# lbarseghyan/diffusion-models

Measured on AMD Instinct MI355X. Metric: sampled images/sec, 32x32 U-Net (dim 64, mults 1-2-4-8), DDPM-1000, higher is better.
Workload: dtype f32; 1 GPU; ddpm1000_32x32_unet64_b256_per_gpu; sampler=p_sample_loop (DDPM), sampler_steps=1000, batch_per_gpu=256, global_batch=256, hip_graph=True, graph_captures=1, parallelism=batch-shard x1, one all-gather per sample()

## Files before the change

### diffusion-models_amd/_lib.py

```python
from __future__ import annotations

import ctypes as C
import os
from typing import Optional

_HERE = os.path.dirname(os.path.abspath(__file__))
LIB_PATH = os.environ.get("DM_LIB") or os.path.join(_HERE, "libdm_hip.so")
DM_MAX_STAGES = 8
DM_COEFS = 8
DM_EDM_COEFS = 16
EDM_HEUN, EDM_DPMPP = 0, 1
DM_CT_COEFS = 16
CT_PRED_NOISE, CT_PRED_V = 0, 1
ABI_VERSION = 9

EXPORTS = (
    "dm_last_error", "dm_abi_version",
    "dm_unet_create", "dm_unet_destroy", "dm_unet_set_param", "dm_unet_missing_params", "dm_unet_get_param_host", "dm_unet_finalize",
    "dm_unet_update_param", "dm_unet_refresh", "dm_unet_graph_captures", "dm_unet_workspace_bytes",
    "dm_unet_forward", "dm_unet_forward_masked", "dm_sample", "dm_sample_cond", "dm_sample_ex", "dm_randn",
    "dm_decoder_create", "dm_decoder_destroy", "dm_decoder_set_param", "dm_decoder_missing_params",
    "dm_decoder_finalize", "dm_decoder_forward",
    "dm_encoder_create", "dm_encoder_destroy", "dm_encoder_set_param", "dm_encoder_missing_params",
    "dm_encoder_finalize", "dm_encoder_forward",
    "dm_op_conv2d", "dm_op_downsample", "dm_op_rmsnorm", "dm_op_block", "dm_op_linear_attention",
    "dm_op_attention", "dm_op_sampler_update", "dm_op_cfg_combine",
    "dm_op_group_norm", "dm_op_vae_attention", "dm_op_vq_nearest",
    "dm_conv_create", "dm_conv_destroy", "dm_conv_forward", "dm_op_pool2d", "dm_op_resize_bilinear",
    "dm_op_copy_channels_nhwc", "dm_op_global_avgpool", "dm_op_linear",
    "dm_unet_train_enable", "dm_unet_grad_floats", "dm_unet_grads_flat", "dm_unet_train_buckets", "dm_unet_train_bucket", "dm_unet_get_grad", "dm_unet_loss_backward", "dm_unet_loss_backward_ex", "dm_unet_loss_backward_masked", "dm_op_q_sample", "dm_op_linear_bwd",
    "dm_op_offset_noise", "dm_op_cdist", "dm_op_gather_rows", "dm_op_lincomb", "dm_op_mask_mix",
    "dm_op_mse_loss", "dm_op_adam_step", "dm_op_ema_lerp",
    "dm_unet_optimizer_step", "dm_unet_train_scalar", "dm_unet_ema_update", "dm_unet_get_param", "dm_unet_set_train_tensor", "dm_unet_adam_step",
    "dm_unet_train_sync", "dm_unet_check_device_pack",
    "dm_unet_train_dropout", "dm_op_dropout_mask",
    "dm_op_conv2d_bwd", "dm_op_downsample_bwd", "dm_op_block_bwd", "dm_op_rmsnorm_bwd", "dm_op_linear_attention_bwd",
    "dm_op_attention_bwd", "dm_op_cross_attention", "dm_op_cross_attention_bwd",
    "dm_profile_enable", "dm_profile_read",
    "dm_unet_forward_ft", "dm_sample_edm",
    "dm_op_edm_churn_in", "dm_op_edm_euler", "dm_op_edm_heun", "dm_op_edm_dpmpp", "dm_op_edm_finalize",
    "dm_unet_train_enable_ft", "dm_unet_loss_backward_edm",
    "dm_op_edm_noise_in", "dm_op_edm_loss", "dm_op_sinusoid_ft_bwd",
    "dm_sample_ct", "dm_unet_loss_backward_ct", "dm_op_ct_step", "dm_op_ct_noise_in", "dm_op_ct_loss",
)


class UnetCfg(C.Structure):
    _fields_ = [
        ("dim", C.c_int32), ("init_dim", C.c_int32), ("out_dim", C.c_int32), ("channels", C.c_int32),
        ("input_channels", C.c_int32), ("n_stages", C.c_int32),
        ("dim_mults", C.c_int32 * DM_MAX_STAGES), ("full_attn", C.c_int32 * DM_MAX_STAGES),
        ("attn_heads", C.c_int32), ("attn_dim_head", C.c_int32),
        ("text_mode", C.c_int32), ("text_emb_dim", C.c_int32), ("sinusoidal_theta", C.c_float),
        ("learned_sinusoidal_dim", C.c_int32), ("attn_heads_stage", C.c_int32 * DM_MAX_STAGES),
    ]


class DecoderCfg(C.Structure):
    _fields_ = [
        ("ch", C.c_int32), ("out_ch", C.c_int32), ("n_levels", C.c_int32), ("ch_mult", C.c_int32 * DM_MAX_STAGES),
        ("num_res_blocks", C.c_int32), ("n_attn_res", C.c_int32), ("attn_resolutions", C.c_int32 * DM_MAX_STAGES),
        ("resolution", C.c_int32), ("z_channels", C.c_int32), ("embed_dim", C.c_int32),
    ]


class EncoderCfg(C.Structure):
    _fields_ = [
        ("ch", C.c_int32), ("in_channels", C.c_int32), ("n_levels", C.c_int32), ("ch_mult", C.c_int32 * DM_MAX_STAGES),
        ("num_res_blocks", C.c_int32), ("n_attn_res", C.c_int32), ("attn_resolutions", C.c_int32 * DM_MAX_STAGES),
        ("resolution", C.c_int32), ("z_channels", C.c_int32), ("embed_dim", C.c_int32), ("n_embed", C.c_int32),
        ("double_z", C.c_int32),
    ]


class SampleArgs(C.Structure):
    _fields_ = [
        ("kind", C.c_int32), ("objective", C.c_int32), ("self_condition", C.c_int32), ("n_steps", C.c_int32),
        ("times_host", C.POINTER(C.c_int64)), ("coefs_host", C.POINTER(C.c_float)),
        ("x_T", C.c_void_p), ("noise", C.c_void_p), ("seed", C.c_uint64), ("sample_offset", C.c_uint64),
        ("ctx", C.c_void_p), ("ctx_tokens", C.c_int32), ("cond_channels", C.c_int32), ("cond", C.c_void_p),
        ("out", C.c_void_p), ("all_steps", C.c_void_p),
        ("B", C.c_int32), ("H", C.c_int32), ("W", C.c_int32), ("unnormalize", C.c_int32), ("use_graph", C.c_int32),
        ("reserved_", C.c_int32), ("stream", C.c_void_p),
        ("cfg", C.c_int32), ("cfg_scale", C.c_float), ("cfg_rescaled_phi", C.c_float),
        ("cfg_keep_parallel_frac", C.c_float), ("cfg_remove_parallel", C.c_int32), ("cfg_reserved_", C.c_int32),
    ]


class EdmArgs(C.Structure):
    _fields_ = [
        ("kind", C.c_int32), ("n_steps", C.c_int32), ("table_host", C.POINTER(C.c_float)),
        ("x_init", C.c_void_p), ("noise", C.c_void_p), ("seed", C.c_uint64), ("sample_offset", C.c_uint64),
        ("out", C.c_void_p), ("sigma_init", C.c_float), ("clamp", C.c_int32),
        ("B", C.c_int32), ("H", C.c_int32), ("W", C.c_int32), ("use_graph", C.c_int32), ("stream", C.c_void_p),
    ]


class EdmTrainArgs(C.Structure):
    _fields_ = [
        ("images", C.c_void_p), ("noise", C.c_void_p), ("coef_host", C.POINTER(C.c_float)), ("coef_stride", C.c_int32),
        ("loss_scale", C.c_float), ("accumulate", C.c_int32), ("B", C.c_int32), ("H", C.c_int32), ("W", C.c_int32),
        ("loss_out_host", C.POINTER(C.c_float)), ("denoised_out", C.c_void_p), ("stream", C.c_void_p),
    ]


class CtArgs(C.Structure):
    _fields_ = [
        ("objective", C.c_int32), ("clip", C.c_int32), ("n_steps", C.c_int32), ("table_host", C.POINTER(C.c_float)),
        ("x_init", C.c_void_p), ("noise", C.c_void_p), ("seed", C.c_uint64), ("sample_offset", C.c_uint64),
        ("out", C.c_void_p), ("B", C.c_int32), ("H", C.c_int32), ("W", C.c_int32), ("use_graph", C.c_int32),
        ("stream", C.c_void_p),
    ]


class CtTrainArgs(C.Structure):
    _fields_ = [
        ("images", C.c_void_p), ("noise", C.c_void_p), ("coef_host", C.POINTER(C.c_float)), ("coef_stride", C.c_int32),
        ("objective", C.c_int32), ("loss_scale", C.c_float), ("accumulate", C.c_int32), ("B", C.c_int32), ("H", C.c_int32),
        ("W", C.c_int32), ("normalize", C.c_int32), ("loss_out_host", C.POINTER(C.c_float)), ("stream", C.c_void_p),
    ]


OBJECTIVES = {"pred_noise": 0, "pred_x0": 1, "pred_v": 2}


class ProfileRow(C.Structure):
    _fields_ = [("kernel", C.c_char * 64), ("launches", C.c_int64), ("total_ms", C.c_double),
                ("total_flops", C.c_double), ("total_bytes", C.c_double)]


_lib: Optional[C.CDLL] = None


def _declare(lib: C.CDLL) -> None:
    vp, i32, i64, u64, fp = C.c_void_p, C.c_int, C.c_int64, C.c_uint64, C.c_void_p
    lib.dm_last_error.restype = C.c_char_p
    lib.dm_last_error.argtypes = []
    lib.dm_abi_version.restype = i32
    lib.dm_unet_create.argtypes = [C.POINTER(UnetCfg), i32, C.POINTER(vp)]
    lib.dm_unet_destroy.argtypes = [vp]
    lib.dm_unet_destroy.restype = None
    lib.dm_unet_set_param.argtypes = [vp, C.c_char_p, fp, C.POINTER(i64), i32]
    lib.dm_unet_missing_params.argtypes = [vp]
    lib.dm_unet_finalize.argtypes = [vp]
    lib.dm_unet_get_param_host.argtypes = [vp, C.c_char_p, vp, i64]
    lib.dm_unet_forward.argtypes = [vp, fp, vp, fp, i32, fp, i32, i32, i32, vp]
    lib.dm_unet_forward_masked.argtypes = [vp, fp, vp, fp, i32, vp, fp, i32, i32, i32, vp]
    lib.dm_unet_update_param.argtypes = [vp, C.c_char_p, fp, C.POINTER(i64), i32]
    lib.dm_unet_refresh.argtypes = [vp]
    lib.dm_unet_graph_captures.argtypes = [vp]
    lib.dm_unet_workspace_bytes.argtypes = [vp]
    lib.dm_unet_workspace_bytes.restype = i64
    lib.dm_sample.argtypes = [vp, i32, i32, C.POINTER(i64), C.POINTER(C.c_float), fp, fp, u64, u64, fp, i32, fp, fp,
                              i32, i32, i32, i32, i32, vp]
    lib.dm_sample_cond.argtypes = [vp, i32, i32, C.POINTER(i64), C.POINTER(C.c_float), fp, fp, u64, u64, fp, i32, fp,
                                   i32, fp, fp, i32, i32, i32, i32, i32, vp]
    lib.dm_sample_ex.argtypes = [vp, C.POINTER(SampleArgs)]
    lib.dm_randn.argtypes = [fp, i64, u64, u64, u64, vp]
    lib.dm_decoder_create.argtypes = [C.POINTER(DecoderCfg), i32, C.POINTER(vp)]
    lib.dm_decoder_destroy.argtypes = [vp]
    lib.dm_decoder_destroy.restype = None
    lib.dm_decoder_set_param.argtypes = [vp, C.c_char_p, fp, C.POINTER(i64), i32]
    lib.dm_decoder_missing_params.argtypes = [vp]
    lib.dm_decoder_finalize.argtypes = [vp]
    lib.dm_decoder_forward.argtypes = [vp, fp, fp, i32, i32, i32, vp]
    lib.dm_encoder_create.argtypes = [C.POINTER(EncoderCfg), i32, C.POINTER(vp)]
    lib.dm_encoder_destroy.argtypes = [vp]
    lib.dm_encoder_destroy.restype = None
    lib.dm_encoder_set_param.argtypes = [vp, C.c_char_p, fp, C.POINTER(i64), i32]
    lib.dm_encoder_missing_params.argtypes = [vp]
    lib.dm_encoder_finalize.argtypes = [vp]
    lib.dm_encoder_forward.argtypes = [vp, fp, fp, fp, vp, i32, i32, i32, vp]
    lib.dm_op_conv2d.argtypes = [fp, i32, fp, i32, fp, fp, fp, fp, i32, i32, i32, i32, i32, i32, i32, vp]
    lib.dm_op_downsample.argtypes = [fp, i32, fp, fp, fp, i32, i32, i32, i32, vp]
    lib.dm_op_rmsnorm.argtypes = [fp, fp, fp, i32, i32, i32, i32, vp]
    lib.dm_op_block.argtypes = [fp, i32, fp, fp, fp, fp, fp, fp, i32, i32, i32, i32, vp]
    lib.dm_op_linear_attention.argtypes = [fp, fp, fp, fp, fp, fp, fp, fp, i32, i32, i32, i32, i32, i32, vp]
    lib.dm_op_attention.argtypes = [fp, fp, fp, fp, fp, fp, fp, i32, i32, i32, i32, i32, i32, vp]
    lib.dm_op_sampler_update.argtypes = [i32, i32, fp, fp, fp, C.POINTER(C.c_float), fp, fp, i64, vp]
    lib.dm_op_cfg_combine.argtypes = [fp, fp, fp, i32, i64, C.c_float, C.c_float, i32, C.c_float, vp]
    lib.dm_op_group_norm.argtypes = [fp, fp, fp, fp, i32, i32, i32, i32, C.c_float, i32, vp]
    lib.dm_op_vae_attention.argtypes = [fp, fp, fp, fp, i32, i32, i32, i32, vp]
    lib.dm_op_vq_nearest.argtypes = [fp, fp, fp, vp, i64, i32, i32, i32, vp]
    lib.dm_conv_create.argtypes = [fp, fp, i32, i32, i32, i32, i32, i32, i32, i32, i32, C.POINTER(vp)]
    lib.dm_conv_destroy.argtypes = [vp]
    lib.dm_conv_destroy.restype = None
    lib.dm_conv_forward.argtypes = [vp, fp, i32, i32, i32, i32, fp, vp]
    lib.dm_op_pool2d.argtypes = [fp, fp, i32, i32, i32, i32, i32, i32, i32, i32, vp]
    lib.dm_op_resize_bilinear.argtypes = [fp, fp, i32, i32, i32, i32, i32, i32, fp, fp, vp]
    lib.dm_op_copy_channels_nhwc.argtypes = [fp, i32, fp, i32, i32, i64, vp]
    lib.dm_op_global_avgpool.argtypes = [fp, fp, i32, i32, i32, vp]
    lib.dm_op_linear.argtypes = [fp, fp, fp, fp, i32, i32, i32, vp]
    lib.dm_unet_train_enable.argtypes = [vp]
    lib.dm_unet_grad_floats.argtypes = [vp]
    lib.dm_unet_grad_floats.restype = i64
    lib.dm_unet_get_grad.argtypes = [vp, C.c_char_p, fp, vp]
    lib.dm_unet_grads_flat.argtypes = [vp, C.POINTER(vp), C.POINTER(i64)]
    lib.dm_unet_train_buckets.argtypes = [vp, i32]
    lib.dm_unet_train_bucket.argtypes = [vp, i32, C.POINTER(i64), C.POINTER(i64), i32, vp]
    lib.dm_unet_loss_backward.argtypes = [vp, fp, C.POINTER(i64), C.POINTER(C.c_float), fp, fp, fp, i32, fp, i32, i32, i32,
                                          C.c_float, i32, C.POINTER(C.c_float), fp, i32, i32, i32, vp]
    lib.dm_unet_loss_backward_ex.argtypes = [vp, C.POINTER(TrainArgs)]
    lib.dm_unet_loss_backward_masked.argtypes = [vp, C.POINTER(TrainArgs), C.POINTER(C.c_int32)]
    lib.dm_unet_optimizer_step.argtypes = [vp, C.c_double, C.c_double, C.c_double, C.c_double, C.c_float, C.POINTER(C.c_float), vp]
    lib.dm_unet_train_scalar.argtypes = [vp, i32, fp, vp]
    lib.dm_unet_ema_update.argtypes = [vp, C.c_double, i32, vp]
    lib.dm_unet_get_param.argtypes = [vp, C.c_char_p, i32, fp, vp]
    lib.dm_unet_set_train_tensor.argtypes = [vp, C.c_char_p, i32, fp, vp]
    lib.dm_unet_adam_step.argtypes = [vp, C.c_longlong]
    lib.dm_unet_adam_step.restype = C.c_longlong
    lib.dm_unet_train_sync.argtypes = [vp]
    lib.dm_unet_train_dropout.argtypes = [vp, C.c_float, u64]
    lib.dm_op_dropout_mask.argtypes = [fp, i64, C.c_float, u64, u64, i32, vp]
    lib.dm_unet_check_device_pack.argtypes = [vp]
    lib.dm_op_q_sample.argtypes = [fp, fp, C.POINTER(C.c_float), fp, i32, i32, vp]
    lib.dm_op_offset_noise.argtypes = [fp, fp, C.c_float, i32, i32, vp]
    lib.dm_op_lincomb.argtypes = [fp, fp, C.POINTER(C.c_float), fp, i32, i64, i32, i32, vp]
    lib.dm_op_mask_mix.argtypes = [fp, fp, fp, fp, i64, vp]
    lib.dm_op_cdist.argtypes = [fp, fp, fp, i32, i32, i64, vp]
    lib.dm_op_gather_rows.argtypes = [fp, C.POINTER(i64), fp, i32, i64, vp]
    lib.dm_op_mse_loss.argtypes = [fp, fp, fp, fp, C.POINTER(C.c_float), i32, i32, C.c_float, C.c_float, fp, C.POINTER(C.c_float),
                                   fp, fp, i32, i32, vp]
    lib.dm_op_adam_step.argtypes = [fp, fp, fp, fp, i64, C.c_double, C.c_double, C.c_double, C.c_double, i32, C.c_float,
                                    C.POINTER(C.c_float), vp]
    lib.dm_op_ema_lerp.argtypes = [fp, fp, i64, C.c_double, vp]
    lib.dm_op_linear_bwd.argtypes = [fp, fp, fp, fp, fp, fp, i32, i32, i32, i32, vp]
    lib.dm_op_conv2d_bwd.argtypes = [fp, i32, fp, i32, fp, fp, fp, fp, fp, fp, i32, i32, i32, i32, i32, i32, i32, vp]
    lib.dm_op_downsample_bwd.argtypes = [fp, i32, fp, fp, fp, fp, fp, i32, i32, i32, i32, vp]
    lib.dm_op_block_bwd.argtypes = [fp, i32] + [fp] * 12 + [i32, i32, i32, i32, vp]
    lib.dm_op_rmsnorm_bwd.argtypes = [fp, fp, fp, fp, fp, i32, i32, i32, i32, vp]
    lib.dm_op_linear_attention_bwd.argtypes = [fp] * 15 + [i32] * 6 + [vp]
    lib.dm_op_attention_bwd.argtypes = [fp] * 13 + [i32] * 6 + [vp]
    lib.dm_op_cross_attention.argtypes = [fp] * 8 + [vp, fp] + [i32] * 7 + [vp]
    lib.dm_op_cross_attention_bwd.argtypes = [fp] * 8 + [vp] + [fp] * 9 + [i32] * 7 + [vp]
    lib.dm_profile_enable.argtypes = [i32]
    lib.dm_unet_forward_ft.argtypes = [vp, fp, fp, fp, i32, fp, i32, i32, i32, vp]
    lib.dm_sample_edm.argtypes = [vp, C.POINTER(EdmArgs)]
    lib.dm_op_edm_churn_in.argtypes = [fp, fp, C.POINTER(C.c_float), i32, u64, u64, u64, fp, fp, i32, i64, vp]
    lib.dm_op_edm_euler.argtypes = [fp, fp, C.POINTER(C.c_float), i32, i32, fp, fp, fp, fp, i32, i64, vp]
    lib.dm_op_edm_heun.argtypes = [fp, fp, fp, fp, C.POINTER(C.c_float), i32, i32, fp, i32, i64, vp]
    lib.dm_op_edm_dpmpp.argtypes = [fp, fp, fp, C.POINTER(C.c_float), i32, fp, i32, i64, vp]
    lib.dm_op_edm_finalize.argtypes = [fp, fp, i64, vp]
    lib.dm_unet_train_enable_ft.argtypes = [vp, i32]
    lib.dm_unet_loss_backward_edm.argtypes = [vp, C.POINTER(EdmTrainArgs)]
    lib.dm_op_edm_noise_in.argtypes = [fp, fp, C.POINTER(C.c_float), i32, fp, fp, fp, i32, i64, vp]
    lib.dm_op_edm_loss.argtypes = [fp, fp, fp, C.POINTER(C.c_float), C.c_float, fp, fp, C.POINTER(C.c_float), i32, i64, vp]
    lib.dm_op_sinusoid_ft_bwd.argtypes = [fp, fp, fp, i32, i32, i32, i32, vp]
    lib.dm_sample_ct.argtypes = [vp, C.POINTER(CtArgs)]
    lib.dm_unet_loss_backward_ct.argtypes = [vp, C.POINTER(CtTrainArgs)]
    lib.dm_op_ct_step.argtypes = [fp, fp, fp, C.POINTER(C.c_float), i32, i32, i32, u64, u64, u64, fp, fp, i32, i64, vp]
    lib.dm_op_ct_noise_in.argtypes = [fp, fp, C.POINTER(C.c_float), i32, i32, i32, fp, fp, i32, i64, vp]
    lib.dm_op_ct_loss.argtypes = [fp, fp, C.POINTER(C.c_float), C.c_float, fp, C.POINTER(C.c_float), i32, i64, vp]
    lib.dm_profile_read.argtypes = [C.POINTER(ProfileRow), i32, C.POINTER(i32)]


class TrainArgs(C.Structure):
    _fields_ = [("x_start", C.c_void_p), ("t_host", C.POINTER(C.c_int64)), ("coef_host", C.POINTER(C.c_float)),
                ("coef_stride", C.c_int), ("noise", C.c_void_p), ("noise_q", C.c_void_p), ("cond", C.c_void_p),
                ("cond_channels", C.c_int), ("ctx", C.c_void_p), ("ctx_tokens", C.c_int), ("self_cond", C.c_int),
                ("objective", C.c_int), ("loss_scale", C.c_float), ("accumulate", C.c_int),
                ("loss_out_host", C.POINTER(C.c_float)), ("model_out", C.c_void_p), ("B", C.c_int), ("H", C.c_int),
                ("W", C.c_int), ("stream", C.c_void_p), ("loss_terms", C.c_int), ("kl_scale", C.c_float)]


def load() -> C.CDLL:
    global _lib
    if _lib is not None:
        return _lib
    if not os.path.exists(LIB_PATH):
        raise RuntimeError(
            f"{LIB_PATH} not found: the HIP extension has not been built. "
            "Run `python -c 'import __graft_entry__ as g; g.build()'` (or `make -C diffusion-models_amd/csrc`). "
            "There is no CPU fallback."
        )
    lib = C.CDLL(LIB_PATH)
    _declare(lib)
    if lib.dm_abi_version() != ABI_VERSION:
        raise RuntimeError(f"libdm_hip.so ABI {lib.dm_abi_version()} != binding ABI {ABI_VERSION}; rebuild")
    _lib = lib
    return lib


def profile_enable(on: bool) -> None:
    check(load().dm_profile_enable(1 if on else 0))


def profile_read():
    rows = (ProfileRow * 64)()
    n = C.c_int(0)
    check(load().dm_profile_read(rows, 64, C.byref(n)))
    return [dict(kernel=rows[i].kernel.decode(), launches=int(rows[i].launches), total_ms=float(rows[i].total_ms),
                 total_flops=float(rows[i].total_flops), total_bytes=float(rows[i].total_bytes))
            for i in range(n.value)]


def check(rc: int) -> None:
    if rc != 0:
        msg = load().dm_last_error().decode(errors="replace")
        raise RuntimeError(f"libdm_hip: {msg}")


def ptr(t) -> Optional[int]:
    if t is None:
        return None
    assert t.is_contiguous(), "tensor must be contiguous at the C ABI"
    return t.data_ptr()
```

### diffusion-models_amd/csrc/conv_device.h

```cpp
#pragma once

#include "dm_common.h"

namespace dm {

using f32x16 = __attribute__((ext_vector_type(16))) float;

__device__ __forceinline__ void block_to_tile(const ConvGeom& g, int bid, int nblk, int& n_tile, int& pblock) {
    n_tile = bid % g.n_tiles_n;
    pblock = bid / g.n_tiles_n;
    if (g.xcd_groups > 0) {
        const int per = (nblk / g.n_tiles_n) / g.xcd_groups;
        pblock = (pblock % g.xcd_groups) * per + pblock / g.xcd_groups;
    }
}
using f32x4 = __attribute__((ext_vector_type(4))) float;
__device__ __forceinline__ f32x4 make_f32x4(float a, float b, float c, float d) { return f32x4{a, b, c, d}; }

using f32x2 = __attribute__((ext_vector_type(2))) float;
__device__ __forceinline__ f32x2 pk_add(f32x2 a, f32x2 b) {
    f32x2 d;
    asm("v_pk_add_f32 %0, %1, %2" : "=v"(d) : "v"(a), "v"(b));
    return d;
}
__device__ __forceinline__ f32x2 pk_sub(f32x2 a, f32x2 b) {
    f32x2 d;
    asm("v_pk_add_f32 %0, %1, %2 neg_lo:[0,1] neg_hi:[0,1]" : "=v"(d) : "v"(a), "v"(b));
    return d;
}
__device__ __forceinline__ f32x2 pk_mul(f32x2 a, f32x2 b) {
    f32x2 d;
    asm("v_pk_mul_f32 %0, %1, %2" : "=v"(d) : "v"(a), "v"(b));
    return d;
}
__device__ __forceinline__ f32x2 pk_fma(f32x2 a, f32x2 b, f32x2 c) {
    f32x2 d;
    asm("v_pk_fma_f32 %0, %1, %2, %3" : "=v"(d) : "v"(a), "v"(b), "v"(c));
    return d;
}
__device__ __forceinline__ f32x4 join4(f32x2 lo, f32x2 hi) { return __builtin_shufflevector(lo, hi, 0, 1, 2, 3); }
__device__ __forceinline__ f32x4 add4(f32x4 a, f32x4 b) { return join4(pk_add(a.xy, b.xy), pk_add(a.zw, b.zw)); }
__device__ __forceinline__ f32x4 sub4(f32x4 a, f32x4 b) { return join4(pk_sub(a.xy, b.xy), pk_sub(a.zw, b.zw)); }
__device__ __forceinline__ f32x4 fma4(f32x4 a, f32x2 s, f32x4 c) {
    return join4(pk_fma(a.xy, s, c.xy), pk_fma(a.zw, s, c.zw));
}

template <int CTRL>
__device__ __forceinline__ float dpp_f(float v) {
    return __builtin_bit_cast(float, __builtin_amdgcn_update_dpp(0, __builtin_bit_cast(int, v), CTRL, 0xF, 0xF, true));
}

__device__ __forceinline__ float half_wave_sum(float v) {
    v += dpp_f<0xB1>(v);
    v += dpp_f<0x4E>(v);
    v += dpp_f<0x141>(v);
    v += dpp_f<0x140>(v);
    v += __builtin_bit_cast(float, __builtin_amdgcn_ds_swizzle(__builtin_bit_cast(int, v), 0x401F));
    return v;
}

__device__ __forceinline__ __amdgpu_buffer_rsrc_t make_rsrc(const float* base, size_t bytes) {
    return __builtin_amdgcn_make_buffer_rsrc(const_cast<float*>(base), 0, (int)min(bytes, (size_t)0xFFFFFFFFu),
                                             0x00020000);
}
__device__ __forceinline__ f32x4 bufload4(__amdgpu_buffer_rsrc_t r, unsigned voff_bytes, unsigned soff_bytes) {
    return __builtin_bit_cast(f32x4, __builtin_amdgcn_raw_buffer_load_b128(r, (int)voff_bytes, (int)soff_bytes, 0));
}

__device__ __forceinline__ float fast_rcp(float x) { return __builtin_amdgcn_rcpf(x); }
__device__ __forceinline__ float fast_rsq(float x) { return __builtin_amdgcn_rsqf(x); }

#ifdef DM_STAMPS
__device__ __forceinline__ unsigned long long dm_stamp_now() {
    unsigned long long t;
    __builtin_amdgcn_sched_barrier(0);
    asm volatile("s_memtime %0\n\ts_waitcnt lgkmcnt(0)" : "=s"(t)::"memory");
    __builtin_amdgcn_sched_barrier(0);
    return t;
}
#define DM_STAMP_DECL unsigned long long st_prev = 0, st_acc[8] = {0, 0, 0, 0, 0, 0, 0, 0};
#define DM_STAMP(k) st_prev = dm_stamp_now();
#define DM_STAMP_ADD(k)                              \
    {                                                \
        unsigned long long st_now = dm_stamp_now();  \
        st_acc[k] += st_now - st_prev;               \
        st_prev = st_now;                            \
    }
#define DM_STAMP_FLUSH                                                                              \
    if (threadIdx.x == 0 && p.stamps) {                                                             \
        unsigned long long* sp_ = p.stamps + ((size_t)blockIdx.y * gridDim.x + blockIdx.x) * 8;     \
        for (int k_ = 0; k_ < 8; ++k_) sp_[k_] = st_acc[k_];                                        \
    }
#else
#define DM_STAMP_DECL
#define DM_STAMP(k)
#define DM_STAMP_ADD(k)
#define DM_STAMP_FLUSH
#endif

struct RowsEpilogue {
    int split;
    size_t M;
    int b0;
    bool uni;
    int HoWo;
    float* red;
    int rows_per_wg;
    int row_in_wg0;
    int wn;
    bool all_valid;
};

using gfloat_ptr = const float __attribute__((address_space(1)))*;
using gfloat_mptr = float __attribute__((address_space(1)))*;
__device__ __forceinline__ f32x4 gload4(gfloat_ptr base, unsigned off_floats) {
    using gchar_ptr = const char __attribute__((address_space(1)))*;
    return *(const f32x4 __attribute__((address_space(1)))*)((gchar_ptr)base + (off_floats << 2));
}
__device__ __forceinline__ void gstore4(gfloat_mptr base, unsigned off_floats, f32x4 v) {
    using gchar_ptr = char __attribute__((address_space(1)))*;
    *(f32x4 __attribute__((address_space(1)))*)((gchar_ptr)base + (off_floats << 2)) = v;
}

template <int NR, bool RES = true>
struct RowsPrefetch {
    f32x4 b4, g4, sc, sh;
    f32x4 res[RES ? NR : 1];
    unsigned off[NR];
};

template <int NR, bool RES>
__device__ __forceinline__ void rows_prefetch(const ConvParams& p, const RowsEpilogue& e, const int (&pixv)[NR], int cg,
                                              bool cvalid, RowsPrefetch<NR, RES>& f) {
    const int cgc = cvalid ? cg : 0;
#pragma unroll
    for (int j = 0; j < NR; ++j) {
        const unsigned px = (unsigned)max(pixv[j], 0);
        f.off[j] = (e.M < (1u << 24) ? __umul24(px, (unsigned)p.Cout) : px * (unsigned)p.Cout) + cgc;
    }
    if (p.partial) return;
    const int epi = p.epi;
    if (epi & EPI_BIAS) f.b4 = *reinterpret_cast<const f32x4*>(p.bias + cgc);
    if (epi & EPI_NORM) f.g4 = *reinterpret_cast<const f32x4*>(p.g + cgc);
    if ((epi & EPI_SCALE_SHIFT) && e.uni) {
        const float* sp = p.scale + (size_t)min(e.b0, p.B - 1) * p.ss_stride;
        f.sc = *reinterpret_cast<const f32x4*>(sp + cgc);
        f.sh = *reinterpret_cast<const f32x4*>(sp + p.Cout + cgc);
    }
    if constexpr (RES) {
        if (epi & EPI_RESIDUAL) {
            const gfloat_ptr rp = (gfloat_ptr)p.residual;
#pragma unroll
            for (int j = 0; j < NR; ++j) f.res[j] = gload4(rp, f.off[j]);
        }
    }
}

template <int WN, int NR, bool RES>
__device__ __forceinline__ void rows_epilogue(const ConvParams& p, const RowsEpilogue& e, f32x4 (&v)[NR],
                                              const int (&pixv)[NR], int cg, bool cvalid,
                                              const RowsPrefetch<NR, RES>& f) {
    const int lane = threadIdx.x & 63;
    const int rsub = lane >> 4;
    if (p.partial) {
        const gfloat_mptr po = (gfloat_mptr)(p.out + (size_t)e.split * e.M * p.Cout);
#pragma unroll
        for (int j = 0; j < NR; ++j)
            if (pixv[j] >= 0 && cvalid) gstore4(po, f.off[j], v[j]);
        return;
    }
    const int epi = p.epi;
    const f32x4 zero4 = make_f32x4(0.f, 0.f, 0.f, 0.f);
    if (epi & EPI_BIAS) {
#pragma unroll
        for (int j = 0; j < NR; ++j) v[j] = add4(v[j], f.b4);
    }
    if (!e.all_valid) {
#pragma unroll
        for (int j = 0; j < NR; ++j) v[j] = cvalid ? v[j] : zero4;
    }
    if (epi & EPI_NORM) {
        const float sqrtc = sqrtf((float)p.Cout);
        const f32x4 g4 = cvalid ? f.g4 * sqrtc : zero4;
        float ssv[NR];
#pragma unroll
        for (int j = 0; j < NR; ++j) {
            const f32x2 sq = pk_fma(v[j].zw, v[j].zw, pk_mul(v[j].xy, v[j].xy));
            float ss = sq.x + sq.y;
            ss += dpp_f<0xB1>(ss);
            ss += dpp_f<0x4E>(ss);
            ss += dpp_f<0x141>(ss);
            ss += dpp_f<0x140>(ss);
            ssv[j] = ss;
        }
        if constexpr (WN > 1) {
            if ((lane & 15) == 0) {
#pragma unroll
                for (int j = 0; j < NR; ++j) e.red[e.wn * e.rows_per_wg + e.row_in_wg0 + 4 * j + rsub] = ssv[j];
            }
            __syncthreads();
#pragma unroll
            for (int j = 0; j < NR; ++j) {
                float t = 0.f;
#pragma unroll
                for (int w = 0; w < WN; ++w) t += e.red[w * e.rows_per_wg + e.row_in_wg0 + 4 * j + rsub];
                ssv[j] = t;
            }
        }
#pragma unroll
        for (int j = 0; j < NR; ++j) {
            const float rn = fast_rsq(fmaxf(ssv[j], 1e-24f));
            const f32x4 gr = g4 * rn;
            v[j] = join4(pk_mul(v[j].xy, gr.xy), pk_mul(v[j].zw, gr.zw));
        }
    }
    if (epi & EPI_SCALE_SHIFT) {
        f32x4 sc = make_f32x4(1.f, 1.f, 1.f, 1.f), sh = zero4;
        if (e.uni) {
            sc = f.sc + 1.0f;
            sh = f.sh;
        }
#pragma unroll
        for (int j = 0; j < NR; ++j) {
            if (!e.uni && cvalid && pixv[j] >= 0) {
                const float* sp = p.scale + (size_t)(pixv[j] / e.HoWo) * p.ss_stride;
                sc = *reinterpret_cast<const f32x4*>(sp + cg) + 1.0f;
                sh = *reinterpret_cast<const f32x4*>(sp + p.Cout + cg);
            }
            v[j] = join4(pk_fma(v[j].xy, sc.xy, sh.xy), pk_fma(v[j].zw, sc.zw, sh.zw));
        }
    }
    if (epi & EPI_SILU) {
        const f32x2 nl2e = {-1.4426950408889634f, -1.4426950408889634f};
#pragma unroll
        for (int j = 0; j < NR; ++j) {
            const f32x2 t0 = pk_mul(v[j].xy, nl2e), t1 = pk_mul(v[j].zw, nl2e);
            f32x4 e4 = make_f32x4(__builtin_amdgcn_exp2f(t0.x), __builtin_amdgcn_exp2f(t0.y),
                                  __builtin_amdgcn_exp2f(t1.x), __builtin_amdgcn_exp2f(t1.y));
            e4 = e4 + 1.0f;
            const f32x4 r4 = make_f32x4(fast_rcp(e4.x), fast_rcp(e4.y), fast_rcp(e4.z), fast_rcp(e4.w));
            v[j] = v[j] * r4;
        }
    }
    if (epi & EPI_RELU) {
#pragma unroll
        for (int j = 0; j < NR; ++j)
            v[j] = make_f32x4(relu_f(v[j].x), relu_f(v[j].y), relu_f(v[j].z), relu_f(v[j].w));
    }
    const gfloat_mptr op = (gfloat_mptr)p.out;
#pragma unroll
    for (int j = 0; j < NR; ++j) {
        if (pixv[j] < 0 || !cvalid) continue;
        if constexpr (RES) {
            gstore4(op, f.off[j], (epi & EPI_RESIDUAL) ? add4(v[j], f.res[j]) : v[j]);
        } else {
            f32x4 r4 = v[j];
            if (epi & EPI_RESIDUAL) r4 = add4(r4, gload4((gfloat_ptr)p.residual, f.off[j]));
            gstore4(op, f.off[j], r4);
        }
    }
}

}
```

### diffusion-models_amd/csrc/dm_api.hip

```cpp
#include "../../include/dm_hip.h"
#include "dm_common.h"
#include "edm.h"
#include "ct.h"

#include <array>
#include <cmath>
#include <cstdlib>
#include <cstring>
#include <functional>
#include <map>
#include <memory>
#include <set>
#include <stdexcept>
#include <string>
#include <unordered_map>
#include <vector>

namespace dm {

static thread_local std::string g_err;
void set_error(const std::string& msg) { g_err = msg; }

namespace prof {
struct Rec {
// ... 529 lines not shown
        return 0;
    }
    std::vector<float> ssw, ssb;
    for (auto& pr : u->resnets) {
        const HostTensor& mw = P(u, pr.first + ".mlp.1.weight");
        const HostTensor& mb = P(u, pr.first + ".mlp.1.bias");
        ssw.insert(ssw.end(), mw.data.begin(), mw.data.end());
        ssb.insert(ssb.end(), mb.data.begin(), mb.data.end());
    }
    if (u->own.upload(ssw.data(), ssw.size(), &u->ss_w) || u->own.upload(ssb.data(), ssb.size(), &u->ss_b)) return 1;
    size_t ow = 0, ob = 0;
    for (auto& pr : u->resnets) {
        const HostTensor& mw = P(u, pr.first + ".mlp.1.weight");
        const HostTensor& mb = P(u, pr.first + ".mlp.1.bias");
        u->own.record_raw(pr.first + ".mlp.1.weight", u->ss_w + ow, mw.data.size());
        u->own.record_raw(pr.first + ".mlp.1.bias", u->ss_b + ob, mb.data.size());
        ow += mw.data.size();
        ob += mb.data.size();
    }
    return 0;
}

static int build_attn_body(dm_unet* u, AttnLayer& A, const std::string& p, int dim, bool full, int heads) {
    A.full = full;
    A.dim = dim;
    A.heads = heads;
    int hidden = heads * u->dh;
    if (up1(u, p + ".norm.g", &A.norm_g) || up1(u, p + ".mem_kv", &A.mem_kv)) return 1;
    conv_src(u, p + ".to_qkv.weight", "");
    if (make_conv(u->own, A.qkv, P(u, p + ".to_qkv.weight").data.data(), nullptr, 3 * hidden, dim, 0, 1, 1, 1, 0, false))
        return 1;
    if (full) {
        conv_src(u, p + ".to_out.weight", p + ".to_out.bias");
        if (make_conv(u->own, A.out, P(u, p + ".to_out.weight").data.data(), P(u, p + ".to_out.bias").data.data(), dim,
                      hidden, 0, 1, 1, 1, 0, false)) return 1;
        A.has16 = false;
        if (attn16_eligible(dim, heads, u->dh)) {
            std::vector<float> wp, wo;
            attn16_pack(P(u, p + ".to_qkv.weight").data.data(), P(u, p + ".norm.g").data.data(),
                        P(u, p + ".to_out.weight").data.data(), dim, wp, wo);
            float *dwp, *dwo;
            if (u->own.upload(wp.data(), wp.size(), &dwp) || u->own.upload(wo.data(), wo.size(), &dwo)) return 1;
            A.a16 = Attn16{dim, dwp, dwo, A.out.bias, A.mem_kv};
            A.has16 = true;
        }
    } else {
        conv_src(u, p + ".to_out.0.weight", p + ".to_out.0.bias");
        if (make_conv(u->own, A.out, P(u, p + ".to_out.0.weight").data.data(), P(u, p + ".to_out.0.bias").data.data(),
                      dim, hidden, 0, 1, 1, 1, 0, false)) return 1;
        if (up1(u, p + ".to_out.1.g", &A.out_g)) return 1;
        if (linattn_fused_eligible(dim, heads, u->dh)) {
            std::vector<float> wq, wk, wv, wo, kb;
            const HostTensor& og = P(u, p + ".to_out.1.g");
            if (linattn_fused_pack(P(u, p + ".to_qkv.weight").data.data(), P(u, p + ".norm.g").data.data(),
                                   P(u, p + ".to_out.0.weight").data.data(), P(u, p + ".mem_kv").data.data(), dim, wq,
                                   wk, wv, wo, kb)) {
                std::vector<float> ogs(og.data);
                for (float& v : ogs) v *= std::sqrt((float)dim);
                float *dq, *dk, *dv, *dwo, *dkb, *dog;
                const HostTensor& wor = P(u, p + ".to_out.0.weight");
                if (u->own.upload(wq.data(), wq.size(), &dq) || u->own.upload(wk.data(), wk.size(), &dk) ||
                    u->own.upload(wv.data(), wv.size(), &dv) || u->own.upload(wor.data.data(), wor.data.size(), &dwo) ||
                    u->own.upload(kb.data(), kb.size(), &dkb) || u->own.upload(ogs.data(), ogs.size(), &dog))
                    return 1;
                A.fused = LinAttnFused{dim, dq, dk, dv, dwo, A.out.bias, dog, dkb, A.mem_kv};
                A.has_fused = true;
            }
        }
    }
    return 0;
}

static int build_attn(dm_unet* u, AttnLayer& A, const std::string& p, int dim, bool full, int heads) {
    return weight_group(u, p, [&]() -> int { return build_attn_body(u, A, p, dim, full, heads); });
}

static int build_cross_body(dm_unet* u, CrossLayer& C, const std::string& p, int dim) {
    int inner = 4 * u->dh;
    conv_src(u, p + ".to_q.weight", "");
    if (make_conv(u->own, C.q, P(u, p + ".to_q.weight").data.data(), nullptr, inner, dim, 0, 1, 1, 1, 0, false)) return 1;
    conv_src(u, p + ".to_out.0.weight", p + ".to_out.0.bias");
    if (make_conv(u->own, C.out, P(u, p + ".to_out.0.weight").data.data(), P(u, p + ".to_out.0.bias").data.data(), dim,
                  inner, 0, 1, 1, 1, 0, false)) return 1;
    if (up1(u, p + ".to_k.weight", &C.wk) || up1(u, p + ".to_v.weight", &C.wv) || up1(u, p + ".to_out.1.g", &C.g) ||
        up1(u, p + ".to_out.0.weight", &C.wo_raw))
        return 1;
    return 0;
}

static int build_cross(dm_unet* u, CrossLayer& C, const std::string& p, int dim) {
    return weight_group(u, p, [&]() -> int { return build_cross_body(u, C, p, dim); });
}

static int build_all(dm_unet* u) {
    const dm_unet_cfg& cfg = u->cfg;
    const int n = cfg.n_stages;
    if (cfg.learned_sinusoidal_dim > 0) {
        if (weight_group(u, "time_mlp.0", [&]() -> int { return up1(u, "time_mlp.0.weights", &u->freqs); })) return 1;
    } else if (weight_group(u, "#freqs", [&]() -> int {
            int half = cfg.dim / 2;
            double k = std::log((double)cfg.sinusoidal_theta) / (half - 1);
            float kf = (float)(-k);
            std::vector<float> f(half);
            for (int i = 0; i < half; ++i) f[i] = std::exp((float)i * kf);
            return u->own.upload(f.data(), f.size(), &u->freqs);
        }))
        return 1;
    if (weight_group(u, "time_mlp", [&]() -> int {
            return up1(u, "time_mlp.1.weight", &u->tw1) || up1(u, "time_mlp.1.bias", &u->tb1) ||
                   up1(u, "time_mlp.3.weight", &u->tw2) || up1(u, "time_mlp.3.bias", &u->tb2);
        }))
        return 1;
    if (weight_group(u, "init_conv", [&]() -> int {
            conv_src(u, "init_conv.weight", "init_conv.bias");
            return make_conv(u->own, u->init_conv, P(u, "init_conv.weight").data.data(), P(u, "init_conv.bias").data.data(),
                             u->init_dim, cfg.input_channels, 0, 7, 7, 1, 3, false);
        }))
        return 1;
    int ss_off = 0;
    u->downs.resize(n);
    u->ups.resize(n);
    for (int i = 0; i < n; ++i) {
        int din = u->dims[i], dout = u->dims[i + 1];
        std::string q = idx("downs", i);
        Stage& S = u->downs[i];
        if (build_resnet(u, S.b1, q + ".0", din, 0, din, ss_off)) return 1;
        if (build_resnet(u, S.b2, q + ".1", din, 0, din, ss_off)) return 1;
        if (build_attn(u, S.attn, q + ".2", din, cfg.full_attn[i] != 0, stage_heads(cfg, i))) return 1;
        if (weight_group(u, q + ".3", [&]() -> int {
                conv_src(u, i < n - 1 ? q + ".3.1.weight" : q + ".3.weight", i < n - 1 ? q + ".3.1.bias" : q + ".3.bias");
                if (i < n - 1) {
                    return make_conv(u->own, S.resample, P(u, q + ".3.1.weight").data.data(),
                                     P(u, q + ".3.1.bias").data.data(), dout, din, 0, 2, 2, 2, 0, false);
                }
                return make_conv(u->own, S.resample, P(u, q + ".3.weight").data.data(), P(u, q + ".3.bias").data.data(),
                                 dout, din, 0, 3, 3, 1, 1, false);
            }))
            return 1;
    }
    int mid = u->dims.back();
    if (build_resnet(u, u->mid1, "mid_block1", mid, 0, mid, ss_off)) return 1;
    if (build_attn(u, u->mid_attn, "mid_attn", mid, true, stage_heads(cfg, n - 1))) return 1;
    if (build_resnet(u, u->mid2, "mid_block2", mid, 0, mid, ss_off)) return 1;
    for (int j = 0; j < n; ++j) {
        int din = u->dims[n - 1 - j], dout = u->dims[n - j];
        std::string q = idx("ups", j);
        Stage& S = u->ups[j];
        if (build_resnet(u, S.b1, q + ".0", dout, din, dout, ss_off)) return 1;
        if (build_resnet(u, S.b2, q + ".1", dout, din, dout, ss_off)) return 1;
        if (build_attn(u, S.attn, q + ".2", dout, cfg.full_attn[n - 1 - j] != 0, stage_heads(cfg, n - 1 - j))) return 1;
        if (weight_group(u, q + ".3", [&]() -> int {
                conv_src(u, j < n - 1 ? q + ".3.1.weight" : q + ".3.weight", j < n - 1 ? q + ".3.1.bias" : q + ".3.bias");
                if (j < n - 1)
                    return make_conv(u->own, S.resample, P(u, q + ".3.1.weight").data.data(),
                                     P(u, q + ".3.1.bias").data.data(), din, dout, 0, 3, 3, 1, 1, true);
                return make_conv(u->own, S.resample, P(u, q + ".3.weight").data.data(), P(u, q + ".3.bias").data.data(),
                                 din, dout, 0, 3, 3, 1, 1, false);
            }))
            return 1;
    }
    if (build_resnet(u, u->final_res, "final_res_block", u->init_dim, u->init_dim, u->init_dim, ss_off)) return 1;
    if (weight_group(u, "final_conv", [&]() -> int {
            conv_src(u, "final_conv.weight", "final_conv.bias");
            return make_conv(u->own, u->final_conv, P(u, "final_conv.weight").data.data(),
                             P(u, "final_conv.bias").data.data(), u->out_dim, u->init_dim, 0, 1, 1, 1, 0, false);
        }))
        return 1;
    u->ss_total = ss_off;
    if (build_scale_shift(u)) return 1;
    if (cfg.text_mode == DM_TEXT_CONCAT) {
        if (weight_group(u, "text_proj", [&]() -> int {
                return up1(u, "text_proj.0.weight", &u->tp_w0) || up1(u, "text_proj.0.bias", &u->tp_b0) ||
                       up1(u, "text_proj.2.weight", &u->tp_w2) || up1(u, "text_proj.2.bias", &u->tp_b2);
            }) ||
            weight_group(u, "text_concat_proj", [&]() -> int {
                return up1(u, "text_concat_proj.weight", &u->tc_w) || up1(u, "text_concat_proj.bias", &u->tc_b);
            }))
            return 1;
    } else if (cfg.text_mode == DM_TEXT_CROSS) {
        if (build_cross(u, u->cross_mid, "cross_attn", mid) || build_cross(u, u->cross_down, "cross_attn_down", mid) ||
            build_cross(u, u->cross_up, "cross_attn_up", mid))
            return 1;
    }
    return 0;
}

struct Ctx {
    dm_unet* u;
    Arena* A;
    hipStream_t s;
    int B;
    const float* ss;
    int ss_stride;
    bool dry() const { return A->dry; }
};

struct ResParts {
    const float* part;
    int nsplit;
    int64_t stride;
    const float* bias;
};

struct PlannedConv {
    ConvParams p;
    int out_h, out_w;
    int kind;
    bool in_kernel;
};

static int plan_conv(const Ctx& c, const ConvLayer& L, bool has_in1, int Hin, int Win, int epi, bool in_nchw, bool out_nchw,
                     PlannedConv& P) {
    ConvParams& p = P.p;
    p = ConvParams{};
    p.C0 = L.C0; p.C1 = L.C1;
    const int CK = conv_ck_for(L.C0, L.C1);
    p.chunks0 = (L.C0 + CK - 1) / CK;
    p.n_chunks = p.chunks0 + (L.C1 ? (L.C1 + CK - 1) / CK : 0);
    p.in_nchw = in_nchw ? 1 : 0;
    p.w = L.w; p.bias = L.bias;
    p.Cout = L.Cout; p.stride = L.stride; p.pad = L.pad;
    const int padw = L.pad_w >= 0 ? L.pad_w : L.pad;
    p.pad_w = padw;
    p.B = c.B;
    p.out_nchw = out_nchw ? 1 : 0;
    p.ss_stride = c.ss_stride;
    const bool want_norm = (epi & EPI_NORM) != 0;
    P.kind = 0;
    const bool upwino = L.up && L.wwu && !in_nchw && !out_nchw && !has_in1 && Hin % 2 == 0 && Win % 2 == 0 &&
                        upwino_shape_ok(c.B, Hin / 2, Win / 2, L.Cout, L.C0, L.C1);
    if (upwino) {
        p.fold = 0; p.fold_w_stride = 0; p.up = 1;
        p.KH = 3; p.KW = 3;
        p.Hin = Hin / 2; p.Win = Win / 2;
        p.Ho = Hin; p.Wo = Win;
        P.out_h = Hin; P.out_w = Win;
        p.w = L.wwu;
        p.chunks0 = p.n_chunks = L.C0 / 8;
        p.geo = upwino_plan(c.B, p.Hin, p.Win, L.Cout, L.C0, L.C1, true);
        P.kind = 3;
    } else if (L.fold) {
        DM_REQUIRE(!out_nchw && !in_nchw, "folded upsample conv is NHWC");
        p.fold = 1; p.fold_w_stride = L.fold_w_stride; p.up = 0;
        p.KH = 2; p.KW = 2; p.pad_w = 1;
        p.Hin = Hin / 2; p.Win = Win / 2;
        p.Ho = p.Hin; p.Wo = p.Win;
        P.out_h = Hin; P.out_w = Win;
        p.geo = conv_plan(c.B, p.Ho, p.Wo, L.Cout, 2, 2, 1, L.C0, L.C1, want_norm, true, 4);
    } else if (L.KH == 2 && L.KW == 2 && L.stride == 2 && L.pad == 0 && !L.up && L.C1 == 0 && L.C0 % 16 == 0 &&
               !in_nchw && Hin % 2 == 0 && Win % 2 == 0) {
        p.fold = 0; p.fold_w_stride = 0; p.up = 0; p.s2d = 1;
        p.KH = 1; p.KW = 1; p.stride = 1; p.pad = 0; p.pad_w = 0;
        p.Ho = Hin / 2; p.Wo = Win / 2;
        p.Hin = p.Ho; p.Win = p.Wo;
        p.chunks0 = p.n_chunks = 4 * (L.C0 / 16);
        P.out_h = p.Ho; P.out_w = p.Wo;
        if (L.wpw && !out_nchw && pw_shape_ok(c.B, p.Ho, p.Wo, L.Cout, 4 * L.C0, 0)) {
            p.w = L.wpw;
            p.geo = pw_plan(c.B, p.Ho, p.Wo, L.Cout, 4 * L.C0, 0, true);
            P.kind = 5;
            P.in_kernel = p.geo.splits == 1 && (!want_norm || p.geo.fused_norm);
            return 0;
        }
        p.geo = conv_plan(c.B, p.Ho, p.Wo, L.Cout, 1, 1, 1, 4 * L.C0, 0, want_norm && !out_nchw, !out_nchw);
    } else {
        p.fold = 0; p.fold_w_stride = 0; p.up = L.up ? 1 : 0;
        p.KH = L.KH; p.KW = L.KW;
        p.Hin = Hin; p.Win = Win;
        p.Ho = (Hin + 2 * L.pad + L.pad_hi - L.KH) / L.stride + 1;
        p.Wo = (Win + 2 * padw + L.pad_hi - L.KW) / L.stride + 1;
        P.out_h = p.Ho; P.out_w = p.Wo;
        p.geo = conv_plan(c.B, p.Ho, p.Wo, L.Cout, L.KH, L.KW, L.stride, L.C0, L.C1, want_norm && !out_nchw,
                          !out_nchw);
    }
    if (P.kind == 0 && L.wi7 && in_nchw && !out_nchw && !has_in1 && epi == 0 && L.pad_hi == 0 && padw == L.pad &&
        (size_t)c.B * p.Ho * p.Wo < (1u << 24)) {
        p.w = L.wi7;
        P.kind = 7;
        P.in_kernel = true;
        return 0;
    }
    if (L.wraw && out_nchw && !in_nchw && !has_in1 && epi == 0) {
        P.kind = 4;
        P.in_kernel = true;
        return 0;
    }
    const bool wino4 = P.kind == 0 && L.ww4 && !L.fold && !in_nchw && !out_nchw && padw == L.pad &&
                       wino4_shape_ok(c.B, p.Ho, p.Wo, L.Cout, L.C0, L.C1);
    const bool wino = P.kind == 0 && !wino4 && L.ww && !L.fold && !in_nchw && !out_nchw && padw == L.pad &&
                      wino_shape_ok(c.B, p.Ho, p.Wo, L.Cout, L.C0, L.C1);
    const bool pw = P.kind == 0 && L.wpw && !L.fold && !p.s2d && !in_nchw && !out_nchw && L.pad_hi == 0 && padw == 0 &&
                    pw_shape_ok(c.B, p.Ho, p.Wo, L.Cout, L.C0, L.C1);
    if (pw) {
        p.w = L.wpw;
        p.chunks0 = L.C0 / 16;
        p.n_chunks = (L.C0 + L.C1) / 16;
        p.geo = pw_plan(c.B, p.Ho, p.Wo, L.Cout, L.C0, L.C1, true);
        P.kind = 5;
    } else if (wino4) {
        p.w = L.ww4;
        p.chunks0 = L.C0 / 8;
        p.n_chunks = (L.C0 + L.C1) / 8;
        p.geo = wino4_plan(c.B, p.Ho, p.Wo, L.Cout, L.C0, L.C1, true);
        P.kind = 2;
    } else if (wino) {
        p.w = L.ww;
        p.chunks0 = L.C0 / 8;
        p.n_chunks = (L.C0 + L.C1) / 8;
        p.geo = wino_plan(c.B, p.Ho, p.Wo, L.Cout, L.C0, L.C1, true, want_norm);
        P.kind = 1;
    }
    P.in_kernel = p.geo.splits == 1 && (!want_norm || p.geo.fused_norm);
    return 0;
}

static int launch_planned(const PlannedConv& P, const ConvParams& q, hipStream_t s, dm_unet* u = nullptr) {
    if (u && u->train && ensure_packed(u, q.w, s)) return 1;
    switch (P.kind) {
        case 7: return init7_launch(q, s);
        case 5: return pw_launch(q, s);
        case 3: return upwino_launch(q, s);
        case 2: return wino4_launch(q, s);
        case 1: return wino_launch(q, s);
        default: return conv_launch(q, s);
    }
}

static int run_conv(Ctx& c, const ConvLayer& L, const float* in0, const float* in1, int Hin, int Win, float* out,
                    int epi, const float* g, const float* scale, const float* residual, bool in_nchw = false,
                    bool out_nchw = false, const ResParts* res_parts = nullptr) {
    PlannedConv P;
    if (plan_conv(c, L, in1 != nullptr, Hin, Win, epi, in_nchw, out_nchw, P)) return 1;
    ConvParams& p = P.p;
    p.in0 = in0; p.in1 = in1;
    p.residual = residual; p.g = g; p.scale = scale;
    if (P.kind == 4) {
        if (c.dry()) return 0;
        if (c.u && c.u->train && ensure_packed(c.u, L.wraw, c.s)) return 1;
        return launch_pointwise_small(in0, L.wraw, L.bias, out, (int64_t)c.B * p.Ho * p.Wo, L.C0, L.Cout, p.Ho * p.Wo,
                                      c.s);
    }
    const int full_epi = epi | (L.bias ? EPI_BIAS : 0);
    if (P.in_kernel) {
        DM_REQUIRE(!res_parts, "residual partial sums need the landing pass");
        if (c.dry()) return 0;
        p.out = out; p.partial = 0; p.epi = full_epi;
        return launch_planned(P, p, c.s, c.u);
    }
    DM_REQUIRE(!out_nchw, "split / unfused epilogue writes NHWC");
    const size_t M = (size_t)c.B * P.out_h * P.out_w;
    float* part = c.A->alloc((size_t)p.geo.splits * M * L.Cout);
    if (c.dry()) {
        c.A->release(part);
        return 0;
    }
    p.out = part; p.partial = 1; p.epi = 0;
    if (launch_planned(P, p, c.s, c.u)) return 1;
    int rc;
    if (res_parts)
        rc = launch_norm_act(part, p.geo.splits, (int64_t)(M * L.Cout), L.bias, g, scale, c.ss_stride, P.out_h * P.out_w,
                             res_parts->part, out, (int64_t)M, L.Cout, full_epi | EPI_RESIDUAL, c.s, res_parts->nsplit,
                             res_parts->stride, res_parts->bias);
    else
        rc = launch_norm_act(part, p.geo.splits, (int64_t)(M * L.Cout), L.bias, g, scale, c.ss_stride, P.out_h * P.out_w,
                             residual, out, (int64_t)M, L.Cout, full_epi, c.s);
    c.A->release(part);
    return rc;
}

static int run_conv_partial(Ctx& c, const ConvLayer& L, const float* in0, const float* in1, int Hin, int Win, float** part,
                            int* nsplit) {
    PlannedConv P;
    if (plan_conv(c, L, in1 != nullptr, Hin, Win, 0, false, false, P)) return 1;
    DM_REQUIRE(P.kind != 4, "partial sums of a pointwise-small layer");
    ConvParams& p = P.p;
    p.in0 = in0; p.in1 = in1;
    const size_t M = (size_t)c.B * P.out_h * P.out_w;
    *part = c.A->alloc((size_t)p.geo.splits * M * L.Cout);
    *nsplit = p.geo.splits;
    if (c.dry()) return 0;
    p.out = *part; p.partial = 1; p.epi = 0;
    return launch_planned(P, p, c.s, c.u);
}

static int run_block(Ctx& c, const ConvLayer& L, const float* in0, const float* in1, int H, int W, const float* g,
                     const float* scale, const float* residual, float* out, const ResParts* res_parts = nullptr) {
    int flags = EPI_NORM | EPI_SILU | (scale ? EPI_SCALE_SHIFT : 0) | (residual ? EPI_RESIDUAL : 0);
    return run_conv(c, L, in0, in1, H, W, out, flags, g, scale, residual, false, false, res_parts);
}

static int run_resnet(Ctx& c, const ResBlock& R, const float* x0, const float* x1, int H, int W, float** out) {
    size_t n = (size_t)c.B * H * W * R.dout;
    const float* scale = c.ss ? c.ss + R.ss_off : nullptr;
    static const bool merge = !env_flag("DM_NO_RES_MERGE");
    PlannedConv P2, Pr;
    bool merged = false;
    if (R.has_res) {
        if (plan_conv(c, R.c2, false, H, W, EPI_NORM | EPI_SILU, false, false, P2)) return 1;
        if (plan_conv(c, R.res, x1 != nullptr, H, W, EPI_RESIDUAL, false, false, Pr)) return 1;
        merged = merge && !P2.in_kernel && !Pr.in_kernel && Pr.kind != 4;
    }
    ResParts rp{};
    float* rpart = nullptr;
    if (merged) {
        if (run_conv_partial(c, R.res, x0, x1, H, W, &rpart, &rp.nsplit)) return 1;
        rp.part = rpart;
        rp.stride = (int64_t)n;
        rp.bias = R.res.bias;
    }
    float* h1 = c.A->alloc(n);
    float* h2 = c.A->alloc(n);
    if (run_block(c, R.c1, x0, x1, H, W, R.g1, scale, nullptr, h1)) return 1;
    if (!R.has_res) {
        if (run_block(c, R.c2, h1, nullptr, H, W, R.g2, nullptr, x0, h2)) return 1;
        c.A->release(h1);
        *out = h2;
        return 0;
    }
    if (merged) {
        if (run_block(c, R.c2, h1, nullptr, H, W, R.g2, nullptr, nullptr, h2, &rp)) return 1;
        c.A->release(rpart);
        c.A->release(h1);
        *out = h2;
        return 0;
    }
    if (run_block(c, R.c2, h1, nullptr, H, W, R.g2, nullptr, nullptr, h2)) return 1;
    c.A->release(h1);
    float* o = c.A->alloc(n);
    if (run_conv(c, R.res, x0, x1, H, W, o, EPI_RESIDUAL, nullptr, nullptr, h2)) return 1;
    c.A->release(h2);
    *out = o;
    return 0;
}

static int run_attn(Ctx& c, const AttnLayer& At, const float* x, int H, int W, float** out, bool add_x = true) {
    const int res_flag = add_x ? EPI_RESIDUAL : 0;
    const float* xres = add_x ? x : nullptr;
    dm_unet* u = c.u;
    const int n = H * W, heads = At.heads, hidden = heads * u->dh;
    const size_t rows = (size_t)c.B * n;
    if (!At.full && At.has_fused) {
        float* ws = c.A->alloc(linattn_fused_ws_floats(c.B, n));
        float* yf = c.A->alloc(rows * At.dim);
        if (!c.dry() && launch_linattn_fused(At.fused, x, ws, yf, c.B, n, add_x, c.s)) return 1;
        c.A->release(ws);
        *out = yf;
        return 0;
    }
    if (At.full && At.has16 && n == 16) {
        float* yf = c.A->alloc(rows * At.dim);
        if (!c.dry() && launch_attn16_fused(At.a16, x, yf, c.B, add_x, c.s)) return 1;
        *out = yf;
        return 0;
    }
    float* xn = c.A->alloc(rows * At.dim);
    float* qkv = c.A->alloc(rows * 3 * hidden);
    float* o = c.A->alloc(rows * hidden);
    float* y = c.A->alloc(rows * At.dim);
    if (!c.dry() && launch_norm_act(x, 1, 0, nullptr, At.norm_g, nullptr, 0, n, nullptr, xn, (int64_t)rows, At.dim,
                                    EPI_NORM, c.s))
        return 1;
    if (run_conv(c, At.qkv, xn, nullptr, H, W, qkv, 0, nullptr, nullptr, nullptr)) return 1;
    if (At.full) {
        if (!c.dry()) {
            const float* mk = At.mem_kv;
            const float* mv = At.mem_kv + (size_t)heads * 4 * u->dh;
            if (launch_attention_core(qkv, 3 * hidden, qkv + hidden, qkv + 2 * hidden, 3 * hidden, mk, mv, 4, o,
                                      hidden, c.B, n, n, heads, u->dh, 1.0f / sqrtf((float)u->dh), c.s))
                return 1;
        }
        if (run_conv(c, At.out, o, nullptr, H, W, y, res_flag, nullptr, nullptr, xres)) return 1;
    } else {
        float* ctxws = c.A->alloc((size_t)c.B * heads * u->dh * u->dh);
        if (!c.dry() && launch_linear_attention_core(qkv, At.mem_kv, ctxws, o, c.B, n, heads, u->dh, c.s)) return 1;
        if (run_conv(c, At.out, o, nullptr, H, W, y, EPI_NORM | res_flag, At.out_g, nullptr, xres)) return 1;
        c.A->release(ctxws);
    }
    c.A->release(xn);
    c.A->release(qkv);
    c.A->release(o);
    *out = y;
    return 0;
}

static bool cross1_off() {
    static const bool off = env_flag("DM_NO_CROSS1");
    return off;
}

static int run_cross(Ctx& c, const CrossLayer& Cr, const float* x, int H, int W, const float* ctx, int m,
                     float** out, const int32_t* tmask = nullptr) {
    auto keep_null_rows = [&](float* y) -> int {
        if (!tmask || c.dry()) return 0;
        return launch_select_rows(y, x, (int64_t)H * W * Cr.out.Cout, tmask, c.B, (int64_t)H * W * Cr.out.Cout, c.s);
    };
    dm_unet* u = c.u;
    const int n = H * W, inner = 4 * u->dh, dim = Cr.out.Cout, E = u->cfg.text_emb_dim;
    const size_t rows = (size_t)c.B * n;
    if (m == 1 && !cross1_off()) {
        float* v = c.A->alloc((size_t)c.B * inner);
        float* yb = c.A->alloc((size_t)c.B * dim);
        float* zb = c.A->alloc((size_t)c.B * dim);
        float* y = c.A->alloc(rows * dim);
        if (!c.dry()) {
            if (launch_linear_rows(ctx, E, Cr.wv, nullptr, v, inner, c.B, E, inner, 0, 0, c.s)) return 1;
            if (launch_linear_rows(v, inner, Cr.wo_raw, Cr.out.bias, yb, dim, c.B, inner, dim, 0, 0, c.s)) return 1;
            if (launch_norm_act(yb, 1, 0, nullptr, Cr.g, nullptr, 0, 1, nullptr, zb, (int64_t)c.B, dim, EPI_NORM, c.s))
                return 1;
            if (launch_broadcast_rows(zb, y, (int)rows, dim, dim, c.s, n)) return 1;
        }
        if (keep_null_rows(y)) return 1;
        c.A->release(v);
        c.A->release(yb);
        c.A->release(zb);
        *out = y;
        return 0;
    }
    float* q = c.A->alloc(rows * inner);
    float* k = c.A->alloc((size_t)c.B * m * inner);
    float* v = c.A->alloc((size_t)c.B * m * inner);
    float* o = c.A->alloc(rows * inner);
    float* y = c.A->alloc(rows * dim);
    if (run_conv(c, Cr.q, x, nullptr, H, W, q, 0, nullptr, nullptr, nullptr)) return 1;
    if (!c.dry()) {
        if (launch_linear_rows(ctx, E, Cr.wk, nullptr, k, inner, c.B * m, E, inner, 0, 0, c.s)) return 1;
        if (launch_linear_rows(ctx, E, Cr.wv, nullptr, v, inner, c.B * m, E, inner, 0, 0, c.s)) return 1;
        if (launch_attention_core(q, inner, k, v, inner, nullptr, nullptr, 0, o, inner, c.B, n, m, 4, u->dh,
                                  1.0f / sqrtf((float)u->dh), c.s))
            return 1;
    }
    if (run_conv(c, Cr.out, o, nullptr, H, W, y, EPI_NORM, Cr.g, nullptr, nullptr)) return 1;
    if (keep_null_rows(y)) return 1;
    c.A->release(q);
    c.A->release(k);
    c.A->release(v);
    c.A->release(o);
    *out = y;
    return 0;
}

static int unet_forward_impl(dm_unet* u, Arena& A, const float* x_nchw, const int64_t* t_dev,
                             const int64_t* step_times, const SamplerState* step_dev, const float* ctx, int ctx_tokens,
                             float* out_nchw, int B, int H, int W, hipStream_t s, const int32_t* tmask = nullptr,
                             const float* tf = nullptr, int tf_stride = 0) {
    const dm_unet_cfg& cfg = u->cfg;
    DM_REQUIRE(!tmask || (ctx && cfg.text_mode != DM_TEXT_NONE), "a text mask needs a text-conditional U-Net and a context");
    Ctx c{u, &A, s, B, nullptr, 0};
    const int td = u->time_dim;
    const bool text_concat = cfg.text_mode == DM_TEXT_CONCAT && ctx != nullptr;
    const bool text_cross = cfg.text_mode == DM_TEXT_CROSS && ctx != nullptr;
    const bool dead_bottleneck = text_cross && ctx_tokens == 1 && !cross1_off() && !tmask;
    const bool shared_t = step_times || (tf && step_dev);
    const int Bt = (shared_t && !text_concat) ? 1 : B;
    const int Rt = shared_t ? 1 : B;
    const int lsd = cfg.learned_sinusoidal_dim;
    const int fdim = lsd > 0 ? lsd + 1 : cfg.dim;
    float* e0 = A.alloc((size_t)Rt * fdim);
    float* e1 = A.alloc((size_t)Rt * td);
    float* temb = A.alloc((size_t)B * td);
    float* ss = A.alloc((size_t)Bt * u->ss_total);
    if (!A.dry) {
        if (tf) {
            if (launch_sinusoid_ft(tf, tf_stride, step_dev, u->freqs, e0, Rt, (lsd > 0 ? lsd : cfg.dim) / 2, s, lsd > 0)) return 1;
        } else if (launch_sinusoid(t_dev, step_times, step_dev, u->freqs, e0, Rt, (lsd > 0 ? lsd : cfg.dim) / 2, s, lsd > 0)) {
            return 1;
        }
        if (launch_linear_rows(e0, fdim, u->tw1, u->tb1, e1, td, Rt, fdim, td, 0, 2, s)) return 1;
        if (launch_linear_rows(e1, td, u->tw2, u->tb2, temb, td, Rt, td, td, 0, 0, s)) return 1;
    }
    const float* tfinal = temb;
    float *cat = nullptr, *tf0 = nullptr;
    if (text_concat) {
        DM_REQUIRE(ctx_tokens == 1, "text concat conditioning takes one pooled embedding per sample");
        cat = A.alloc((size_t)B * 2 * td);
        tf0 = A.alloc((size_t)B * td);
        float* t2 = A.alloc((size_t)B * td);
        if (!A.dry) {
            if (Rt == 1) {
                if (launch_broadcast_rows(temb, cat, B, td, 2 * td, s)) return 1;
            } else {
                DM_CHECK_HIP(hipMemcpy2DAsync(cat, 2 * td * sizeof(float), temb, td * sizeof(float),
                                              td * sizeof(float), B, hipMemcpyDeviceToDevice, s));
            }
            if (launch_linear_rows(ctx, cfg.text_emb_dim, u->tp_w0, u->tp_b0, tf0, td, B, cfg.text_emb_dim, td, 0, 2, s))
                return 1;
            if (launch_linear_rows(tf0, td, u->tp_w2, u->tp_b2, cat + td, 2 * td, B, td, td, 0, 0, s)) return 1;
            if (launch_linear_rows(cat, 2 * td, u->tc_w, u->tc_b, t2, td, B, 2 * td, td, 0, 0, s)) return 1;
            if (tmask && launch_select_rows(t2, temb, Rt == 1 ? 0 : td, tmask, B, td, s)) return 1;
        }
        tfinal = t2;
    }
    if (!A.dry) {
        if (launch_linear_rows(tfinal, td, u->ss_w, u->ss_b, ss, u->ss_total, Bt, td, u->ss_total, 1, 0, s)) return 1;
    }
    c.ss = A.dry ? reinterpret_cast<const float*>(16) : ss;
    c.ss_stride = Bt == 1 ? 0 : u->ss_total;

    const int n_st = cfg.n_stages;
    float* x = A.alloc((size_t)B * H * W * u->init_dim);
    if (run_conv(c, u->init_conv, x_nchw, nullptr, H, W, x, 0, nullptr, nullptr, nullptr, true)) return 1;
    if (cat) A.release(cat);
    if (tf0) A.release(tf0);
    if (tfinal != temb) A.release(tfinal);
    A.release(e0);
    A.release(e1);
    A.release(temb);
    const float* r = x;
    auto rel = [&](const float* t) {
        if (t != r) A.release(t);
    };
    std::vector<const float*> skips;
    int h = H, w = W;
    float* cur = x;
    for (int i = 0; i < n_st; ++i) {
        Stage& S = u->downs[i];
        float *a, *b2, *at;
        if (run_resnet(c, S.b1, cur, nullptr, h, w, &a)) return 1;
        rel(cur);
        skips.push_back(a);
        if (run_resnet(c, S.b2, a, nullptr, h, w, &b2)) return 1;
        if (run_attn(c, S.attn, b2, h, w, &at)) return 1;
        rel(b2);
        skips.push_back(at);
        int ho = (i < n_st - 1) ? h / 2 : h, wo = (i < n_st - 1) ? w / 2 : w;
        if (i == n_st - 1 && dead_bottleneck) {
            cur = nullptr;
            break;
        }
        float* d = A.alloc((size_t)B * ho * wo * S.resample.Cout);
        if (run_conv(c, S.resample, at, nullptr, h, w, d, 0, nullptr, nullptr, nullptr)) return 1;
        cur = d; h = ho; w = wo;
    }
    float* t0;
    if (dead_bottleneck) {
        if (run_cross(c, u->cross_up, nullptr, h, w, ctx, ctx_tokens, &t0)) return 1;
        cur = t0;
    } else {
        if (text_cross) { if (run_cross(c, u->cross_down, cur, h, w, ctx, ctx_tokens, &t0, tmask)) return 1; rel(cur); cur = t0; }
        if (run_resnet(c, u->mid1, cur, nullptr, h, w, &t0)) return 1; rel(cur); cur = t0;
        if (text_cross) { if (run_cross(c, u->cross_mid, cur, h, w, ctx, ctx_tokens, &t0, tmask)) return 1; rel(cur); cur = t0; }
        if (run_attn(c, u->mid_attn, cur, h, w, &t0)) return 1; rel(cur); cur = t0;
        if (run_resnet(c, u->mid2, cur, nullptr, h, w, &t0)) return 1; rel(cur); cur = t0;
        if (text_cross) { if (run_cross(c, u->cross_up, cur, h, w, ctx, ctx_tokens, &t0, tmask)) return 1; rel(cur); cur = t0; }
    }
    for (int j = 0; j < n_st; ++j) {
        Stage& S = u->ups[j];
        float *a, *b2, *at;
        const float* sk = skips.back(); skips.pop_back();
        if (run_resnet(c, S.b1, cur, sk, h, w, &a)) return 1;
        rel(cur);
        rel(sk);
        sk = skips.back(); skips.pop_back();
        if (run_resnet(c, S.b2, a, sk, h, w, &b2)) return 1;
        rel(a);
        rel(sk);
        if (run_attn(c, S.attn, b2, h, w, &at)) return 1;
        rel(b2);
        bool last = j == n_st - 1;
        int ho = last ? h : h * 2, wo = last ? w : w * 2;
        float* d = A.alloc((size_t)B * ho * wo * S.resample.Cout);
        if (run_conv(c, S.resample, at, nullptr, ho, wo, d, 0, nullptr, nullptr, nullptr)) return 1;
        rel(at);
        cur = d; h = ho; w = wo;
    }
    float* fr;
    if (run_resnet(c, u->final_res, cur, r, h, w, &fr)) return 1;
    rel(cur);
    A.release(r);
    if (run_conv(c, u->final_conv, fr, nullptr, h, w, out_nchw, 0, nullptr, nullptr, nullptr, false, true))
        return 1;
    A.release(fr);
    A.release(ss);
    return 0;
}

static int ensure_workspace(dm_unet* u, size_t bytes) {
    if (bytes <= u->ws_cap) return 0;
    DM_CHECK_HIP(hipDeviceSynchronize());
    u->drop_graph();
    if (u->ws) (void)hipFree(u->ws);
    u->ws = nullptr;
    u->ws_cap = 0;
    void* p = nullptr;
    DM_CHECK_HIP(hipMalloc(&p, bytes));
    u->ws = static_cast<char*>(p);
// ... 506 lines not shown
```

### diffusion-models_amd/csrc/dm_common.h

```cpp
#pragma once

#include <hip/hip_runtime.h>
#include <stdint.h>

#include <string>
#include <vector>

#include <cstdlib>

namespace dm {

inline int env_int(const char* name, int dflt) {
    const char* e = std::getenv(name);
    return e ? std::atoi(e) : dflt;
}
inline bool env_flag(const char* name) { return std::getenv(name) != nullptr; }

__device__ __forceinline__ float relu_f(float v) { return v < 0.0f ? 0.0f : v; }

void set_error(const std::string& msg);

#define DM_CHECK_HIP(expr)                                                                  \
    do {                                                                                    \
        hipError_t _e = (expr);                                                             \
        if (_e != hipSuccess) {                                                             \
            dm::set_error(std::string(#expr) + ": " + hipGetErrorString(_e));               \
            return 1;                                                                       \
        }                                                                                   \
    } while (0)

#define DM_REQUIRE(cond, msg)                                                               \
    do {                                                                                    \
        if (!(cond)) {                                                                      \
            dm::set_error(std::string(msg) + " [" #cond "]");                                \
            return 1;                                                                       \
        }                                                                                   \
    } while (0)

struct LdsOptIn {
    unsigned char done[64] = {};
};
inline int lds_opt_in(LdsOptIn& f, const void* kernel, int n_kernels) {
    int dev = 0;
    DM_CHECK_HIP(hipGetDevice(&dev));
    const bool tracked = dev >= 0 && dev < 64;
    if (tracked && f.done[dev] >= n_kernels) return 0;
    DM_CHECK_HIP(hipFuncSetAttribute(kernel, hipFuncAttributeMaxDynamicSharedMemorySize, 160 * 1024));
    if (tracked) ++f.done[dev];
    return 0;
}


enum ConvEpilogue : int {
    EPI_BIAS = 1,
    EPI_NORM = 2,
    EPI_SCALE_SHIFT = 4,
    EPI_SILU = 8,
    EPI_RESIDUAL = 16,
    EPI_RELU = 32,
};

struct ConvGeom {
    int WM, WN;
    int CK;
    int TW, TH, NB;
    int lTW, lTH;
    int tiles_x, tiles_y, groups, n_tiles_n;
    int IH, IW;
    int halo_floats;
    int w_floats;
    int ptab_off;
    int TPS;
    int splits;
    int chunks_per_split;
    int fused_norm;
    int row_stride;
    int magic_win, magic_row;
    int lds_bytes;
    int xcd_groups;
    int NQ;
};

struct ConvParams {
    const float* in0;
    const float* in1;
    int C0, C1;
    int chunks0;
    int n_chunks;
    int Hin, Win;
    int up;
    int in_nchw;
    const float* w;
    const float* bias;
    int Cout, KH, KW, stride, pad;
    int pad_w;
    int B, Ho, Wo;
    float* out;
    int out_nchw;
    int partial;
    int fold;
    int s2d;
    int fold_w_stride;
    unsigned long long* stamps;
    int epi;
    const float* residual;
    const float* g;
    const float* scale;
    int ss_stride;
    ConvGeom geo;
};

ConvGeom conv_plan(int B, int Ho, int Wo, int Cout, int KH, int KW, int stride, int C0, int C1, bool want_norm,
                   bool allow_split, int grid_z = 1);
int conv_ck_for(int C0, int C1);
size_t conv_packed_floats(int Cout, int C0, int C1, int KH, int KW);
void conv_pack_weights(const float* oihw, float* packed, int Cout, int C0, int C1, int KH, int KW);
int conv_launch(const ConvParams& p, hipStream_t s);

bool winograd_off();
bool wino_eligible(int Cout, int C0, int C1, int KH, int KW, int stride, int pad, bool up);
size_t wino_packed_floats(int Cout, int C0, int C1);
void wino_pack_weights(const float* oihw, float* packed, int Cout, int C0, int C1);
ConvGeom wino_plan(int B, int Ho, int Wo, int Cout, int C0, int C1, bool allow_split, bool want_norm = true);
bool wino_shape_ok(int B, int Ho, int Wo, int Cout, int C0, int C1);
int wino_launch(const ConvParams& p, hipStream_t s);

bool wino4_eligible(int Cout, int C0, int C1, int KH, int KW, int stride, int pad, bool up);
size_t wino4_packed_floats(int Cout, int C0, int C1);
void wino4_pack_weights(const float* oihw, float* packed, int Cout, int C0, int C1);
ConvGeom wino4_plan(int B, int Ho, int Wo, int Cout, int C0, int C1, bool allow_split);
bool wino4_shape_ok(int B, int Ho, int Wo, int Cout, int C0, int C1);
int wino4_launch(const ConvParams& p, hipStream_t s);

bool init7_eligible(int Cout, int C0, int C1, int KH, int KW, int stride, int pad, bool up);
size_t init7_packed_floats(int Cin);
void init7_pack_weights(const float* oihw, float* packed, int Cin);
int init7_launch(const ConvParams& p, hipStream_t s);

bool pw_eligible(int Cout, int C0, int C1, int KH, int KW, int stride, int pad, bool up);
size_t pw_packed_floats(int Cout, int C0, int C1);
void pw_pack_weights(const float* oihw, float* packed, int Cout, int C0, int C1);
bool pw_s2d_eligible(int Cout, int C0, int C1, int KH, int KW, int stride, int pad, bool up);
void pw_pack_weights_s2d(const float* oihw, float* packed, int Cout, int C0);
ConvGeom pw_plan(int B, int Ho, int Wo, int Cout, int C0, int C1, bool allow_split);
bool pw_shape_ok(int B, int Ho, int Wo, int Cout, int C0, int C1);
int pw_launch(const ConvParams& p, hipStream_t s);

struct Attn16 {
    int C;
    const float* wp;
    const float* wo;
    const float* bias;
    const float* mem_kv;
};
bool attn16_eligible(int dim, int heads, int dh);
void attn16_pack(const float* w_qkv, const float* norm_g, const float* w_out, int C, std::vector<float>& wp,
                 std::vector<float>& wo);
int launch_attn16_fused(const Attn16& w, const float* x, float* y, int B, bool add_x, hipStream_t s);

bool upwino_eligible(int Cout, int C0, int C1, int KH, int KW, int stride, int pad, bool up);
size_t upwino_packed_floats(int Cout, int C0, int C1);
void upwino_pack_weights(const float* oihw, float* packed, int Cout, int C0, int C1);
ConvGeom upwino_plan(int B, int Hl, int Wl, int Cout, int C0, int C1, bool allow_split);
bool upwino_shape_ok(int B, int Hl, int Wl, int Cout, int C0, int C1);
int upwino_launch(const ConvParams& p, hipStream_t s);

namespace prof {
bool enabled();
bool detail();
int begin(const char* kernel, double flops, double bytes, hipStream_t s);
int end(hipStream_t s);
}

int launch_nchw_to_nhwc(const float* in, float* out, int B, int C, int HW, hipStream_t s);
int launch_nhwc_to_nchw(const float* in, float* out, int B, int C, int HW, hipStream_t s);
int launch_norm_act(const float* x, int nsplit, int64_t split_stride, const float* bias, const float* g,
                    const float* scale, int ss_stride, int pix_per_image, const float* residual, float* y,
                    int64_t rows, int C, int flags, hipStream_t s, int res_nsplit = 1, int64_t res_stride = 0,
                    const float* res_bias = nullptr);
int launch_linear_rows(const float* x, int ldx, const float* W, const float* bias, float* y, int ldy, int R, int I,
                       int O, int act_in, int act_out, hipStream_t s);
struct SamplerState {
    int step;
    int n_steps;
    int unnormalize;
    int pad_;
    uint64_t seed;
    uint64_t off4;
};
int launch_sinusoid(const int64_t* t, const int64_t* step_times, const SamplerState* step, const float* freqs, float* e,
                    int R, int half, hipStream_t s, bool learned = false);
bool vae_attn_mfma_ok(int n, int C);
int launch_vae_attn_mfma(const float* q, const float* k, const float* v, float* out, int B, int n, int C, hipStream_t s);
bool group_sums_ok(int C, int groups);
size_t group_stats_ws_floats(int B, int groups);
int launch_group_stats_fast(const float* x, float* stats, double* acc, int B, int HW, int C, int groups, float eps,
                            hipStream_t s);
int launch_group_norm(const float* x, const float* w, const float* b, float* y, float* stats_ws, int B, int HW,
                      int C, int groups, float eps, int swish, hipStream_t s);
int launch_add(const float* a, const float* b, float* y, int64_t n, hipStream_t s);
int launch_pool2d_nhwc(const float* in, float* out, int B, int H, int W, int C, int k, int stride, int pad, int mode,
                       hipStream_t s);
int launch_resize_bilinear(const float* in_nchw, float* out_nhwc, int B, int C, int H, int W, int Ho, int Wo,
                           const float* scale, const float* shift, hipStream_t s);
int launch_copy_channels_nhwc(const float* src, int Cs, float* dst, int Cd, int c_off, int64_t rows, hipStream_t s);
int launch_global_avgpool_nhwc(const float* in, float* out, int B, int HW, int C, hipStream_t s);
int launch_spin(double milliseconds, hipStream_t s);
int launch_copy_channels(const float* src, float* dst, int B, int Cs, int Cd, int c_off, int HW, hipStream_t s);
int launch_pointwise_small(const float* x, const float* w_oc, const float* bias, float* y_nchw, int64_t pixels, int C,
                           int Cout, int HW, hipStream_t s);

int launch_sampler_update(int kind, const float* x, const float* eps, const float* noise, const float* coefs_dev,
                          const SamplerState* state_dev, int64_t noise_step_stride, float* out, float* all_steps,
                          float* final_out, int64_t n, hipStream_t s, int objective = 0, float* xstart_out = nullptr,
                          float* dup_out = nullptr);
int launch_randn(float* out, int64_t n, uint64_t seed, uint64_t draw, uint64_t element_offset, hipStream_t s);
int launch_step_advance(SamplerState* state_dev, hipStream_t s);
int launch_finalize(const float* x, float* out, int64_t n, int unnormalize, hipStream_t s);
int launch_broadcast_rows(const float* src, float* dst, int rows, int n, int ld, hipStream_t s, int group = 0);

struct CfgParams {
    float cond_scale, rescaled_phi, keep_parallel_frac, remove_parallel;
};
int launch_cfg_combine(const float* cond, const float* null_out, float* out, int B, int64_t per, const float* params_dev,
                       CfgParams p, hipStream_t s);
int launch_select_rows(float* y, const float* x, int64_t x_ld, const int32_t* mask, int B, int64_t per, hipStream_t s);
int launch_route_rows(float* dst, int64_t dst_ld, const float* kept, int64_t kept_ld, const float* dropped,
                      int64_t dropped_ld, const int32_t* mask, int B, int64_t per, hipStream_t s);

int launch_linear_attention_core(const float* qkv, const float* mem_kv, float* ctx_ws, float* out, int B, int n,
                                 int heads, int dh, hipStream_t s, float* kstats = nullptr);
int launch_attention_core(const float* q, int ldq, const float* k, const float* v, int ldk, const float* mem_k,
                          const float* mem_v, int n_mem, float* out, int ldo, int B, int nq, int nk, int heads,
                          int dh, float scale, hipStream_t s);

struct LinAttnFused {
    int C;
    const float *wq, *wk, *wv;
    const float* wo_raw;
    const float* bias;
    const float* og;
    const float* kbound;
    const float* mem_kv;
};
bool linattn_fused_eligible(int C, int heads, int dh);
bool linattn_fused_pack(const float* w_qkv, const float* norm_g, const float* w_out, const float* mem_kv, int C,
                        std::vector<float>& wq, std::vector<float>& wk, std::vector<float>& wv, std::vector<float>& wo,
                        std::vector<float>& kbound);
size_t linattn_fused_ws_floats(int B, int n);
int launch_linattn_fused(const LinAttnFused& w, const float* x, float* ws, float* y, int B, int n, bool add_x,
                         hipStream_t s);


size_t wgrad_ws_floats(int B, int Ho, int Wo, int Cout, int Cin, int T, int* splits_out);
struct WgradJob {
    const float* partial;
    float* out;
    long long oc;
    int splits, T, accumulate, first_block;
};
int launch_wgrad(const float* in0, int C0, const float* in1, int C1, const float* dy, int Cout, int B, int Ho, int Wo,
                 int mode, int up, float* ws, float* dw, int accumulate, hipStream_t s, WgradJob* defer = nullptr);
struct WgradParams {
    const float* in0;
    const float* in1;
    const float* dy;
    float* partial;
    int C0, C1, Cin, Cout;
    int B, Ho, Wo;
    int up;
    int TW, R, NB;
    int tiles_x, tiles_y;
    int n_blocks, blocks_per_split;
    int n_ct, n_kt;
    int n_splits, first_wg;
};
struct WgradDesc {
    const float *in0, *in1, *dy;
    float* dw;
    int C0, C1, Cout, B, Ho, Wo, up, accumulate;
};
void wgrad_group_plan(const std::vector<WgradDesc>& descs, int mode, std::vector<int>& splits, std::vector<size_t>& ws_floats);
int wgrad_group_fill(const std::vector<WgradDesc>& descs, int mode, const std::vector<int>& splits, const std::vector<float*>& ws,
                     std::vector<WgradParams>& table, std::vector<WgradJob>& jobs, int* total_wgs, size_t* lds_bytes);
int launch_wgrad_group(const WgradParams* table_dev, int n_jobs, int total_wgs, size_t lds_bytes, int mode, hipStream_t s);
size_t thin_out_bwd_ws_floats(int B, int H, int W, int Cout, int Cin);
bool thin_out_bwd_ok(int Cout, int HW);
int launch_thin_out_bwd(const float* x, const float* dy_nchw, const float* w_oc, float* dx, float* ws, float* dw, float* db,
                        int B, int H, int W, int Cin, int Cout, int accumulate, hipStream_t s, WgradJob* defer_w,
                        WgradJob* defer_b);
size_t wgrad_naive_ws_floats(int B, int H, int Cout, int Cin, int KH, int KW, int* splits_out);
int launch_wgrad_naive(const float* x, int x_nchw, const float* dy, int dy_nchw, int Cin, int Cout, int KH, int KW, int pad,
                       int B, int H, int W, float* ws, float* dw, int accumulate, hipStream_t s, WgradJob* defer = nullptr);
int launch_wgrad_reduce_jobs(const WgradJob* jobs_dev, int n_jobs, int total_blocks, hipStream_t s);
int wgrad_reduce_pairs(int T, long long oc);
size_t norm_act_bwd_ws_floats(int B, int pix_per_image, int C);
struct RowgradJob {
    const float* part;
    float *dss, *img, *dg, *dbias;
    int chunks, C, dss_stride, B, accumulate, first_img_block, first_fin_block;
    int pad_;
};
struct ColsumJob {
    const float* x;
    float *ws, *out;
    long long rows, row_stride, col_stride;
    int C, accumulate, nb, rpb, first_part_block, first_fin_block;
};
int launch_norm_act_bwd(const float* dy, const float* u, const float* g, const float* ss, int ss_stride, int pix_per_image,
                        float* du, float* ws, float* dg, float* dbias, float* dss, int dss_stride, int B, int C, int flags,
                        int accumulate, hipStream_t s, RowgradJob* defer = nullptr, float drop_p = 0.f, uint64_t drop_seed = 0,
                        uint64_t drop_stream = 0, const float* add = nullptr, int dy_nsplit = 1, int64_t dy_stride = 0);
int launch_norm_act_drop(const float* u, const float* g, const float* ss, int ss_stride, int pix_per_image, const float* residual,
                         float* y, int B, int C, int flags, float drop_p, uint64_t drop_seed, uint64_t drop_stream, hipStream_t s,
                         int nsplit = 1, int64_t split_stride = 0, const float* bias = nullptr, float* u_out = nullptr);
void rowgrad_jobs_prefix(std::vector<RowgradJob>& jobs, int* img_blocks, int* fin_blocks);
int launch_rowgrad_jobs(const RowgradJob* jobs_dev, int n_jobs, int img_blocks, int fin_blocks, hipStream_t s);
void colsum_jobs_prefix(std::vector<ColsumJob>& jobs, int* part_blocks, int* fin_blocks);
int launch_colsum_jobs(const ColsumJob* jobs_dev, int n_jobs, int n_with_partial, int part_blocks, int fin_blocks, hipStream_t s);
size_t colsum_ws_floats(int64_t rows, int C);
int launch_colsum(const float* x, int64_t rows, int C, int64_t row_stride, int64_t col_stride, float* ws, float* out,
                  int accumulate, hipStream_t s, ColsumJob* defer = nullptr);
int launch_colsum_nchw(const float* dy, int B, int C, int HW, float* out, int accumulate, hipStream_t s);
int launch_act_fwd(const float* x, float* y, int64_t n, int act, hipStream_t s);
int launch_act_bwd(const float* dy, const float* x, float* dx, int64_t n, int act, hipStream_t s);
int launch_add3(const float* a, const float* b, const float* c, float* y, int64_t n, hipStream_t s);
int launch_dropout(const float* x, const float* add, float* out, int64_t n, float p, uint64_t seed, uint64_t stream,
                   hipStream_t s);
int launch_depth_to_space(const float* t, const float* add, float* dx, int B, int Ho, int Wo, int C, hipStream_t s);
int launch_pool2x2_sum(const float* du, const float* add, float* dx, int B, int H, int W, int C, hipStream_t s);
int launch_pointwise_small_dgrad(const float* dy_nchw, const float* w_oc, float* dx, int64_t pixels, int C, int Cout, int HW,
                                 hipStream_t s);
int launch_linear_wgrad(const float* dy, int ldy, const float* x, int ldx, float* dw, int R, int I, int O, int act_in,
                        int accumulate, hipStream_t s);
int launch_mlp_rows_wgrad(const float* dy, int ldy, const float* x, int ldx, float* const* dw_rows, float* const* db_rows,
                          int R, int I, int O, int accumulate, hipStream_t s, const float* x_act = nullptr);
int launch_lincomb(const float* x, const float* y, const float* coef_dev, float* out, int B, int64_t per_sample, int mode,
                   int clamp, hipStream_t s);
int launch_mask_mix(const float* a, const float* b, const float* mask, float* out, int64_t n, hipStream_t s);
int launch_offset_noise(float* noise, const float* offset, float strength, int BC, int HW, hipStream_t s);
int launch_cdist(const float* x, const float* y, float* out, int n, int m, int64_t D, hipStream_t s);
size_t linear_dgrad_ws_floats(int R, int I, int O);
bool small_gemm_off();
bool rows_gemm_nt_ok(int R, int I, int O, int ldx);
int launch_rows_gemm_nt(const float* x, int ldx, const float* W, const float* bias, float* y, int ldy, int R, int I, int O,
                        hipStream_t s);
bool rows_gemm_nn_ok(int R, int I, int O, int ldy, int ldx);
int rows_gemm_nn_shares(int O);
int launch_rows_gemm_nn(const float* dy, int ldy, const float* W, float* dx_or_ws, int ldx, int R, int I, int O, hipStream_t s);
bool rows_gemm_tn_ok(int R, int I, int O, int ldy, int ldx);
int launch_rows_gemm_tn(const float* dy, int ldy, const float* x, int ldx, float* const* dw_rows, float* const* db_rows, float* dw,
                        int ldw, float* db, int R, int I, int O, int accumulate, hipStream_t s);
int launch_linear_dgrad(const float* dy, int ldy, const float* W, float* dx, int ldx, int R, int I, int O, float* ws,
                        hipStream_t s);
#define DM_TRAIN_COEFS 12
int launch_pred_x_start(const float* x, const float* out, const float* coef_dev, float* xs, int B, int per_sample, int objective,
                        hipStream_t s);
int launch_q_sample(const float* x_start, const float* noise, const float* coef_dev, float* x, int B, int per_sample,
                    hipStream_t s);
int launch_mse_loss(const float* out, const float* x_start, const float* noise, const float* coef_dev, float* dout,
                    float* part, float* loss, int B, int per_sample, int objective, float loss_scale, hipStream_t s,
                    int terms = 1, const float* xq = nullptr, float* klpart = nullptr, float kl_scale = 0.f);
int launch_lerp(float* ema, const float* p, int64_t n, double decay, hipStream_t s);
int launch_pack_direct(const float* oihw, float* packed, int Cout, int C0, int C1, int KH, int KW, hipStream_t s);
int launch_fold_taps(const float* oihw, float* w2, int Cout, int Cin, int py, int px, hipStream_t s);
int launch_pack_wino(const float* oihw, float* packed, int Cout, int Cin, hipStream_t s);
int launch_pack_wino4(const float* oihw, float* packed, int Cout, int Cin, hipStream_t s);
int launch_pack_upwino(const float* oihw, float* packed, int Cout, int Cin, hipStream_t s);
int launch_pack_pw(const float* w, float* packed, int Cout, int Cin, int s2d_C0, hipStream_t s);
int launch_pack_init7(const float* oihw, float* packed, int Cin, hipStream_t s);
enum PackJobKind { PJ_COPY = 0, PJ_ROT, PJ_S2D_T, PJ_WINO, PJ_WINO4, PJ_UPWINO, PJ_PW };
struct PackJob {
    const float* src;
    float* dst;
    long long n;
    int kind, Cout, Cin, a, b, first_block;
    int rs = 0, rc = 0;
};
int pack_jobs_prefix(std::vector<PackJob>& jobs);
int launch_pack_jobs(const PackJob* jobs_dev, int n_jobs, int total_blocks, hipStream_t s);
int launch_rot_transpose(const float* w, float* out, int Cout, int Cin, int K, int c_lo, int c_n, hipStream_t s);
int launch_s2d_transpose(const float* w, float* out, int Cout, int C, hipStream_t s);
int launch_scatter_copy(const float* param, const void* table_dev, int n_entries, long long max_n, hipStream_t s);
int launch_grad_norm(const float* grads, int64_t n, double* part_ws, float max_norm, float* out2, hipStream_t s);
int launch_adam(float* p, const float* g, float* m, float* v, const double* coef, int64_t n, double lr, double b1, double b2,
                double eps, int step, hipStream_t s);
size_t linattn_bwd_ws_floats(int B, int n, int heads, int dh);
int launch_linear_attention_core_bwd(const float* qkv, const float* mem_kv, const float* ctx, const float* dout, float* ws,
                                     float* dqkv, float* dmem_part, int B, int n, int heads, int dh, hipStream_t s,
                                     const float* kstats);
size_t attn_bwd_ws_floats(int B, int nq, int nk, int n_mem, int heads, int dh);
int launch_attention_core_bwd(const float* qkv, const float* mem_kv, const float* dout, float* dqkv, float* dmem_part, float* ws,
                              int B, int n, int heads, int dh, hipStream_t s);
int launch_cross_attention_core_bwd(const float* q, const float* k, const float* v, const float* dout, float* dq, float* dk,
                                    float* dv, float* ws, int B, int nq, int m, int heads, int dh, hipStream_t s);

}
```

### diffusion-models_amd/csrc/dm_ops.inc

```
namespace dm {

static int d2h(const float* dev, size_t n, std::vector<float>& out) {
    out.resize(n);
    if (n) DM_CHECK_HIP(hipMemcpy(out.data(), dev, n * sizeof(float), hipMemcpyDeviceToHost));
    return 0;
}

template <class F>
static int run_op(hipStream_t s, F body) {
    Arena dry;
    dry.dry = true;
    if (body(dry)) return 1;
    void* buf = nullptr;
    DM_CHECK_HIP(hipMalloc(&buf, dry.off + 256));
    Arena A;
    A.base = static_cast<char*>(buf);
    A.cap = dry.off + 256;
    int rc = body(A);
    hipError_t e = hipStreamSynchronize(s);
    (void)hipFree(buf);
    if (!rc && e != hipSuccess) {
        set_error(std::string("kernel execution failed: ") + hipGetErrorString(e));
        rc = 1;
    }
    return rc;
}

static float* to_nhwc(Arena& A, const float* nchw, int B, int C, int HW, hipStream_t s, int* rc) {
    float* t = A.alloc((size_t)B * C * HW);
    if (!A.dry && launch_nchw_to_nhwc(nchw, t, B, C, HW, s)) *rc = 1;
    return t;
}

static void init_dummy(dm_unet& u, int heads, int dh) {
    u.heads = heads;
    u.dh = dh;
    u.cfg.attn_heads = heads;
    u.cfg.attn_dim_head = dh;
}

}

extern "C" {

int dm_op_conv2d(const float* in0, int C0, const float* in1, int C1, const float* weight, const float* bias,
                 const float* residual, float* out, int B, int H, int W, int Cout, int ksize, int pad, int up2,
                 void* stream) {
    DM_REQUIRE(in0 && weight && out, "null argument");
    hipStream_t s = static_cast<hipStream_t>(stream);
    std::vector<float> wh, bh;
    if (d2h(weight, (size_t)Cout * (C0 + C1) * ksize * ksize, wh)) return 1;
    if (bias && d2h(bias, Cout, bh)) return 1;
    dm_unet dummy;
    init_dummy(dummy, 4, 32);
    ConvLayer L;
    if (make_conv(dummy.own, L, wh.data(), bias ? bh.data() : nullptr, Cout, C0, in1 ? C1 : 0, ksize, ksize, 1, pad,
                  up2 != 0)) return 1;
    const int Hin = up2 ? 2 * H : H, Win = up2 ? 2 * W : W;
    const int Ho = Hin + 2 * pad - ksize + 1, Wo = Win + 2 * pad - ksize + 1;
    return run_op(s, [&](Arena& A) -> int {
        int rc = 0;
        Ctx c{&dummy, &A, s, B, nullptr, 0};
        if (L.wi7 && !in1 && !residual && !up2) {
            float* o = A.alloc((size_t)B * Ho * Wo * Cout);
            if (run_conv(c, L, in0, nullptr, Hin, Win, o, 0, nullptr, nullptr, nullptr, true)) return 1;
            if (!A.dry && launch_nhwc_to_nchw(o, out, B, Cout, Ho * Wo, s)) return 1;
            return 0;
        }
        float* a0 = to_nhwc(A, in0, B, C0, H * W, s, &rc);
        float* a1 = in1 ? to_nhwc(A, in1, B, C1, H * W, s, &rc) : nullptr;
        float* r = residual ? to_nhwc(A, residual, B, Cout, Ho * Wo, s, &rc) : nullptr;
        float* o = A.alloc((size_t)B * Ho * Wo * Cout);
        if (rc) return 1;
        if (run_conv(c, L, a0, a1, Hin, Win, o, residual ? EPI_RESIDUAL : 0, nullptr, nullptr, r)) return 1;
        if (!A.dry && launch_nhwc_to_nchw(o, out, B, Cout, Ho * Wo, s)) return 1;
        return 0;
    });
}

int dm_op_downsample(const float* in, int C, const float* weight, const float* bias, float* out, int B, int H,
                     int W, int Cout, void* stream) {
    DM_REQUIRE(in && weight && out, "null argument");
    DM_REQUIRE(H % 2 == 0 && W % 2 == 0, "downsample needs even H, W");
    hipStream_t s = static_cast<hipStream_t>(stream);
    std::vector<float> wh, bh;
    if (d2h(weight, (size_t)Cout * 4 * C, wh)) return 1;
    if (bias && d2h(bias, Cout, bh)) return 1;
    dm_unet dummy;
    init_dummy(dummy, 4, 32);
    ConvLayer L;
    if (make_conv(dummy.own, L, wh.data(), bias ? bh.data() : nullptr, Cout, C, 0, 2, 2, 2, 0, false)) return 1;
    return run_op(s, [&](Arena& A) -> int {
        int rc = 0;
        Ctx c{&dummy, &A, s, B, nullptr, 0};
        float* a0 = to_nhwc(A, in, B, C, H * W, s, &rc);
        float* o = A.alloc((size_t)B * (H / 2) * (W / 2) * Cout);
        if (rc) return 1;
        if (run_conv(c, L, a0, nullptr, H, W, o, 0, nullptr, nullptr, nullptr)) return 1;
        if (!A.dry && launch_nhwc_to_nchw(o, out, B, Cout, (H / 2) * (W / 2), s)) return 1;
        return 0;
    });
}

int dm_op_rmsnorm(const float* x, const float* g, float* out, int B, int C, int H, int W, void* stream) {
    DM_REQUIRE(x && g && out, "null argument");
    hipStream_t s = static_cast<hipStream_t>(stream);
    return run_op(s, [&](Arena& A) -> int {
        int rc = 0;
        float* a = to_nhwc(A, x, B, C, H * W, s, &rc);
        float* o = A.alloc((size_t)B * C * H * W);
        if (rc) return 1;
        if (A.dry) return 0;
        if (launch_norm_act(a, 1, 0, nullptr, g, nullptr, 0, H * W, nullptr, o, (int64_t)B * H * W, C, EPI_NORM, s))
            return 1;
        return launch_nhwc_to_nchw(o, out, B, C, H * W, s);
    });
}

int dm_op_block(const float* x, int Cin, const float* weight, const float* bias, const float* g, const float* scale,
                const float* shift, float* out, int B, int H, int W, int Cout, void* stream) {
    DM_REQUIRE(x && weight && bias && g && out, "null argument");
    DM_REQUIRE((scale == nullptr) == (shift == nullptr), "scale and shift come together");
    hipStream_t s = static_cast<hipStream_t>(stream);
    std::vector<float> wh, bh;
    if (d2h(weight, (size_t)Cout * Cin * 9, wh) || d2h(bias, Cout, bh)) return 1;
    dm_unet dummy;
    init_dummy(dummy, 4, 32);
    ConvLayer L;
    if (make_conv(dummy.own, L, wh.data(), bh.data(), Cout, Cin, 0, 3, 3, 1, 1, false)) return 1;
    return run_op(s, [&](Arena& A) -> int {
        int rc = 0;
        Ctx c{&dummy, &A, s, B, nullptr, 0};
        float* a = to_nhwc(A, x, B, Cin, H * W, s, &rc);
        float* ss = nullptr;
        if (scale) {
            ss = A.alloc((size_t)B * 2 * Cout);
            if (!A.dry) {
                DM_CHECK_HIP(hipMemcpy2DAsync(ss, 2 * Cout * sizeof(float), scale, Cout * sizeof(float),
                                              Cout * sizeof(float), B, hipMemcpyDeviceToDevice, s));
                DM_CHECK_HIP(hipMemcpy2DAsync(ss + Cout, 2 * Cout * sizeof(float), shift, Cout * sizeof(float),
                                              Cout * sizeof(float), B, hipMemcpyDeviceToDevice, s));
            }
            c.ss_stride = 2 * Cout;
        }
        float* o = A.alloc((size_t)B * H * W * Cout);
        if (rc) return 1;
        const float* sc = scale ? (A.dry ? reinterpret_cast<const float*>(16) : ss) : nullptr;
        if (run_block(c, L, a, nullptr, H, W, g, sc, nullptr, o)) return 1;
        if (!A.dry && launch_nhwc_to_nchw(o, out, B, Cout, H * W, s)) return 1;
        return 0;
    });
}

static int attn_op(bool full, const float* x, const float* norm_g, const float* mem_kv, const float* w_qkv,
                   const float* w_out, const float* b_out, const float* out_g, float* out, int B, int C, int H,
                   int W, int heads, int dim_head, void* stream) {
    DM_REQUIRE(x && norm_g && mem_kv && w_qkv && w_out && b_out && out, "null argument");
    DM_REQUIRE(dim_head == 32 || dim_head == 64, "dim_head: the attention kernels support 32 and 64");
    hipStream_t s = static_cast<hipStream_t>(stream);
    const int hidden = heads * dim_head;
    std::vector<float> wq, wo, bo;
    if (d2h(w_qkv, (size_t)3 * hidden * C, wq) || d2h(w_out, (size_t)C * hidden, wo) || d2h(b_out, C, bo)) return 1;
    dm_unet dummy;
    init_dummy(dummy, heads, dim_head);
    AttnLayer At;
    At.full = full;
    At.dim = C;
    At.heads = heads;
    At.norm_g = const_cast<float*>(norm_g);
    At.mem_kv = const_cast<float*>(mem_kv);
    At.out_g = const_cast<float*>(out_g);
    if (make_conv(dummy.own, At.qkv, wq.data(), nullptr, 3 * hidden, C, 0, 1, 1, 1, 0, false)) return 1;
    if (make_conv(dummy.own, At.out, wo.data(), bo.data(), C, hidden, 0, 1, 1, 1, 0, false)) return 1;
    return run_op(s, [&](Arena& A) -> int {
        int rc = 0;
        Ctx c{&dummy, &A, s, B, nullptr, 0};
        float* a = to_nhwc(A, x, B, C, H * W, s, &rc);
        if (rc) return 1;
        float* y = nullptr;
        if (run_attn(c, At, a, H, W, &y, false)) return 1;
        if (!A.dry && launch_nhwc_to_nchw(y, out, B, C, H * W, s)) return 1;
        return 0;
    });
}

int dm_op_linear_attention(const float* x, const float* norm_g, const float* mem_kv, const float* w_qkv,
                           const float* w_out, const float* b_out, const float* out_g, float* out, int B, int C,
                           int H, int W, int heads, int dim_head, void* stream) {
    DM_REQUIRE(out_g, "null argument");
    return attn_op(false, x, norm_g, mem_kv, w_qkv, w_out, b_out, out_g, out, B, C, H, W, heads, dim_head, stream);
}

int dm_op_attention(const float* x, const float* norm_g, const float* mem_kv, const float* w_qkv,
                    const float* w_out, const float* b_out, float* out, int B, int C, int H, int W, int heads,
                    int dim_head, void* stream) {
    return attn_op(true, x, norm_g, mem_kv, w_qkv, w_out, b_out, nullptr, out, B, C, H, W, heads, dim_head, stream);
}

int dm_profile_enable(int on) {
    prof::g_on = on != 0;
    prof::g_detail = on == 2;
    if (on) {
        constexpr int N = 33;
        hipEvent_t e0[N], e1[N];
        for (int i = 0; i < N; ++i) {
            DM_CHECK_HIP(hipEventCreate(&e0[i]));
            DM_CHECK_HIP(hipEventCreate(&e1[i]));
        }
        if (launch_spin(2.0, nullptr)) return 1;
        for (int i = 0; i < N; ++i) {
            DM_CHECK_HIP(hipEventRecord(e0[i], nullptr));
            if (launch_spin(0.0, nullptr)) return 1;
            DM_CHECK_HIP(hipEventRecord(e1[i], nullptr));
        }
        DM_CHECK_HIP(hipDeviceSynchronize());
        std::vector<float> ms(N);
        for (int i = 0; i < N; ++i) {
            DM_CHECK_HIP(hipEventElapsedTime(&ms[i], e0[i], e1[i]));
            (void)hipEventDestroy(e0[i]);
            (void)hipEventDestroy(e1[i]);
        }
        std::sort(ms.begin(), ms.end());
        prof::g_overhead_ms = ms[N / 2];
    }
    return 0;
}

int dm_profile_read(dm_profile_row* rows, int max_rows, int* n_rows) {
    DM_REQUIRE(rows && n_rows && max_rows > 0, "bad argument");
    DM_CHECK_HIP(hipDeviceSynchronize());
    std::map<std::string, dm_profile_row> agg;
    for (auto& r : prof::g_recs) {
        float ms = 0.f;
        DM_CHECK_HIP(hipEventElapsedTime(&ms, r.e0, r.e1));
        dm_profile_row& a = agg[r.kernel];
        if (a.launches == 0) {
            std::memset(&a, 0, sizeof(a));
            std::snprintf(a.kernel, sizeof(a.kernel), "%s", r.kernel.c_str());
        }
        a.launches += 1;
        a.total_ms += std::max(0.0, (double)ms - prof::g_overhead_ms);
        a.total_flops += r.flops;
        a.total_bytes += r.bytes;
        prof::g_pool.push_back(r.e0);
        prof::g_pool.push_back(r.e1);
    }
    prof::g_recs.clear();
    int n = 0;
    for (auto& kv : agg) {
        if (n >= max_rows) break;
        rows[n++] = kv.second;
    }
    *n_rows = n;
    return 0;
}

int dm_op_sampler_update(int kind, int objective, const float* x, const float* eps, const float* noise,
                         const float* c_host, float* out, float* x_start, int64_t n, void* stream) {
    DM_REQUIRE(x && eps && c_host && out, "null argument");
    DM_REQUIRE(objective >= DM_OBJ_PRED_NOISE && objective <= DM_OBJ_PRED_V, "unknown objective");
    hipStream_t s = static_cast<hipStream_t>(stream);
    float* cd = nullptr;
    DM_CHECK_HIP(hipMalloc(reinterpret_cast<void**>(&cd), DM_COEFS * sizeof(float)));
    DM_CHECK_HIP(hipMemcpy(cd, c_host, DM_COEFS * sizeof(float), hipMemcpyHostToDevice));
    int rc = launch_sampler_update(kind, x, eps, noise, cd, nullptr, 0, out, nullptr, nullptr, n, s, objective, x_start);
    hipError_t e = hipStreamSynchronize(s);
    (void)hipFree(cd);
    if (!rc && e != hipSuccess) {
        set_error(std::string("kernel execution failed: ") + hipGetErrorString(e));
        rc = 1;
    }
    return rc;
}

int dm_op_cfg_combine(const float* cond, const float* null_out, float* out, int B, int64_t per_sample, float cond_scale,
                      float rescaled_phi, int remove_parallel_component, float keep_parallel_frac, void* stream) {
    DM_REQUIRE(cond && null_out && out, "null argument");
    DM_REQUIRE(B > 0 && per_sample > 1, "dm_op_cfg_combine needs B > 0 and more than one value per sample");
    DM_REQUIRE(out != cond && out != null_out, "dm_op_cfg_combine does not run in place");
    DM_REQUIRE(remove_parallel_component == 0 || remove_parallel_component == 1, "remove_parallel_component is 0 or 1");
    const CfgParams p{cond_scale, rescaled_phi, keep_parallel_frac, (float)remove_parallel_component};
    return launch_cfg_combine(cond, null_out, out, B, per_sample, nullptr, p, static_cast<hipStream_t>(stream));
}

}
```

### diffusion-models_amd/csrc/wino4_mfma.hip

```cpp
#include "conv_device.h"

#include <algorithm>
#include <cstdio>
#include <cstdlib>
#include <type_traits>
#include <vector>

namespace dm {

static constexpr int W4CK = 8;
static constexpr int W4TILES = 16;
static constexpr int W4WTS = 68;


template <int LTW>
struct W4Geo {
    static constexpr int TW = 1 << LTW;
    static constexpr int TH = TW;
    static constexpr int NB = W4TILES / (TW * TH);
    static constexpr int IH = 4 * TH + 2, IW = 4 * TW + 2;
    static constexpr int RS = ((IW * W4CK + 63) / 64) * 64;
    static constexpr int BUF = NB * IH * RS;
    static constexpr int HR = LTW == 2 ? 3 : 2;
};
__host__ __device__ constexpr int w4_nbcode(int ltw, int nb) {
    return ltw == 2 ? 0 : (ltw == 1 ? ((nb & 1) | ((nb & 2) << 1)) : (nb & 15));
}

bool wino4_eligible(int Cout, int C0, int C1, int KH, int KW, int stride, int pad, bool up) {
    static const bool off = env_flag("DM_NO_WINO4") || winograd_off();
    return !off && KH == 3 && KW == 3 && stride == 1 && pad == 1 && !up && C0 > 0 && C0 % W4CK == 0 &&
           C1 % W4CK == 0 && Cout % 64 == 0;
}

size_t wino4_packed_floats(int Cout, int C0, int C1) { return (size_t)(C0 + C1) * 36 * Cout; }

static inline int w4_index(int h, int t) {
    static const int lo[3] = {0, 1, 2}, hi[3] = {5, 3, 4};
    return h ? hi[t] : lo[t];
}

void wino4_pack_weights(const float* oihw, float* packed, int Cout, int C0, int C1) {
    static const double G[6][3] = {{0.25, 0, 0},           {-1.0 / 6, -1.0 / 6, -1.0 / 6}, {-1.0 / 6, 1.0 / 6, -1.0 / 6},
                                   {1.0 / 24, 1.0 / 12, 1.0 / 6}, {1.0 / 24, -1.0 / 12, 1.0 / 6}, {0, 0, 1}};
    const int Cin = C0 + C1;
    for (int co = 0; co < Cout; ++co)
        for (int ci = 0; ci < Cin; ++ci) {
            const float* gk = oihw + ((size_t)co * Cin + ci) * 9;
            double Gg[6][3];
            for (int i = 0; i < 6; ++i)
                for (int b = 0; b < 3; ++b) Gg[i][b] = G[i][0] * gk[b] + G[i][1] * gk[3 + b] + G[i][2] * gk[6 + b];
            double U[6][6];
            for (int i = 0; i < 6; ++i)
                for (int j = 0; j < 6; ++j) U[i][j] = Gg[i][0] * G[j][0] + Gg[i][1] * G[j][1] + Gg[i][2] * G[j][2];
            const int chunk = ci / W4CK, cc = ci % W4CK;
            for (int g = 0; g < 4; ++g)
                for (int a = 0; a < 3; ++a)
                    for (int b = 0; b < 3; ++b) {
                        const int i = w4_index(g >> 1, a), j = w4_index(g & 1, b);
                        const int ct = co / 64, gq = (co % 64) / 16, n = co % 16, kq = cc / 2, st = cc % 2;
                        packed[(((((size_t)chunk * 4 + g) * 9 + a * 3 + b) * (Cout / 64) + ct) * 4 + kq) * 128 + n * 8 +
                               gq * 2 + st] = (float)U[i][j];
                    }
        }
}

static int w4_class(int Ho, int Wo) {
    if (Ho == 4 && Wo == 4) return 0;
    if (Ho == 8 && Wo == 8) return 1;
    if (Wo % 16 == 0 && Ho % 16 == 0 && Ho > 0 && Wo > 0) return 2;
    return -1;
}

ConvGeom wino4_plan(int B, int Ho, int Wo, int Cout, int C0, int C1, bool allow_split) {
    ConvGeom g{};
    const int ltw = w4_class(Ho, Wo);
    g.WM = 1;
    g.WN = 1;
    g.CK = W4CK;
    g.lTW = ltw < 0 ? 0 : ltw;
    g.TW = 1 << g.lTW;
    g.TH = g.TW;
    g.lTH = g.lTW;
    g.NB = W4TILES / (g.TW * g.TH);
    g.tiles_x = std::max(1, Wo / (4 * g.TW));
    g.tiles_y = std::max(1, Ho / (4 * g.TH));
    g.groups = (B + g.NB - 1) / g.NB;
    g.n_tiles_n = Cout / 64;
    g.IH = 4 * g.TH + 2;
    g.IW = 4 * g.TW + 2;
    g.row_stride = ((g.IW * W4CK + 63) / 64) * 64;
    g.halo_floats = g.NB * g.IH * g.row_stride;
    g.TPS = 3;
    const int n_chunks = (C0 + C1) / W4CK;
    const int wgs = g.tiles_x * g.tiles_y * g.groups * g.n_tiles_n;
    int splits = 1;
    if (allow_split) {
        static const int target = env_int("DM_WINO4_TARGET_WGS", 256);
        static const int min_chunks = env_int("DM_WINO4_MIN_CHUNKS", 8);
        while (wgs * splits < target && splits < 8 && n_chunks / (splits * 2) >= min_chunks) splits *= 2;
    }
    g.chunks_per_split = (n_chunks + splits - 1) / splits;
    g.splits = (n_chunks + g.chunks_per_split - 1) / g.chunks_per_split;
    g.fused_norm = g.n_tiles_n == 1 && g.splits == 1;
    g.w_floats = 0;
    g.ptab_off = std::max(3 * g.halo_floats + 16, 2 * 12 * W4TILES * W4WTS);
    g.lds_bytes = (g.ptab_off + 16 * W4TILES) * 4;
    return g;
}

bool wino4_shape_ok(int B, int Ho, int Wo, int Cout, int C0, int C1) {
    if (w4_class(Ho, Wo) < 0) return false;
    const ConvGeom g = wino4_plan(B, Ho, Wo, Cout, C0, C1, true);
    static const int min_wgs = env_int("DM_WINO4_MIN_WGS", 200);
    static const int min_k = env_int("DM_WINO4_MIN_K", 12);
    const int wgs = g.tiles_x * g.tiles_y * g.groups * g.n_tiles_n * g.splits;
    return wgs >= min_wgs && g.chunks_per_split >= min_k && g.lds_bytes <= 160 * 1024 &&
           (size_t)B * Ho * Wo < (1u << 24) && (size_t)B * Ho * Wo * std::max(C0, C1) < (1ull << 30);
}

__device__ __forceinline__ f32x2 pk_fma_s(f32x2 sa, f32x2 b, f32x2 c) {
    f32x2 d;
    asm("v_pk_fma_f32 %0, %1, %2, %3" : "=v"(d) : "s"(sa), "v"(b), "v"(c));
    return d;
}
__device__ __forceinline__ f32x2 pk_fms_s(f32x2 sa, f32x2 b, f32x2 c) {
    f32x2 d;
    asm("v_pk_fma_f32 %0, %1, %2, %3 neg_lo:[1,0,0] neg_hi:[1,0,0]" : "=v"(d) : "s"(sa), "v"(b), "v"(c));
    return d;
}
__device__ __forceinline__ f32x2 pk_mul_s(f32x2 sa, f32x2 b) {
    f32x2 d;
    asm("v_pk_mul_f32 %0, %1, %2" : "=v"(d) : "s"(sa), "v"(b));
    return d;
}

struct W4Coef {
    f32x2 k, l, pe, p0, p1, p2, p3;
};
__device__ __forceinline__ W4Coef w4_coef(int hi) {
    W4Coef c;
    const float k = hi ? 1.f : 4.f, l = hi ? 2.f : 1.f, pe = hi ? 1.f : 4.f;
    const float p0 = hi ? 4.f : 0.f, p1 = hi ? 0.f : -5.f, p2 = hi ? -5.f : 0.f, p3 = hi ? 0.f : 1.f;
    c.k = f32x2{k, k};
    c.l = f32x2{l, l};
    c.pe = f32x2{pe, pe};
    c.p0 = f32x2{p0, p0};
    c.p1 = f32x2{p1, p1};
    c.p2 = f32x2{p2, p2};
    c.p3 = f32x2{p3, p3};
    return c;
}
__device__ __forceinline__ void w4_half(const W4Coef& c, f32x2 e, f32x2 z0, f32x2 z1, f32x2 z2, f32x2 z3, f32x2& oP,
                                        f32x2& oPlus, f32x2& oMinus) {
    const f32x2 S = pk_fms_s(c.k, z1, z3);
    const f32x2 D = pk_fms_s(c.k, z0, z2);
    oPlus = pk_fma_s(c.l, D, S);
    oMinus = pk_fms_s(c.l, D, S);
    f32x2 t = pk_mul_s(c.pe, e);
    t = pk_fma_s(c.p0, z0, t);
    t = pk_fma_s(c.p1, z1, t);
    t = pk_fma_s(c.p2, z2, t);
    oP = pk_fma_s(c.p3, z3, t);
}

template <int LTW>
__global__ __launch_bounds__(256, 1) void wino4_mfma_kernel(const ConvParams p) {
    using G = W4Geo<LTW>;
    constexpr int TW = G::TW, TH = G::TH, NB = G::NB, IH = G::IH, IW = G::IW, RS = G::RS, BUF = G::BUF, HR = G::HR;
    extern __shared__ __attribute__((aligned(16))) float smem[];
    const ConvGeom& g = p.geo;
    const int tid = threadIdx.x;
    const int lane = tid & 63;
    const int wave = __builtin_amdgcn_readfirstlane(tid >> 6);
    const int RT = wave >> 1, CT = wave & 1;
    const int l15 = lane & 15;
    const int kq = lane >> 4;

    int n_tile, bid;
    block_to_tile(g, blockIdx.x, gridDim.x, n_tile, bid);
    const int tile_x = bid % g.tiles_x;
    bid /= g.tiles_x;
    const int tile_y = bid % g.tiles_y;
    const int group = bid / g.tiles_y;
    const int tx0 = tile_x * TW, ty0 = tile_y * TH, b0 = group * NB;
    const int ix0 = 4 * tx0 - 1, iy0 = 4 * ty0 - 1;
    const int split = blockIdx.y;
    const int cb = split * g.chunks_per_split;
    const int ce = min(cb + g.chunks_per_split, p.n_chunks);
    float* raw[2] = {smem, smem + BUF};
    DM_STAMP_DECL
    DM_STAMP(0);
    constexpr int SCRATCH = 2 * BUF;

    int hpix[HR], hoff[HR];
#pragma unroll
    for (int i = 0; i < HR; ++i) {
        const int it = tid + 256 * i;
        const int hp = it >> 1, qd = it & 1;
        int nb, hy, hx;
        bool in_region;
        if constexpr (LTW == 2) {
            hy = hp / IW;
            hx = hp - hy * IW;
            nb = 0;
            in_region = hp < IH * IW;
        } else {
            constexpr int PIX = 16 * TW * TH;
            nb = hp / PIX;
            const int r = hp - nb * PIX;
            hy = r / (4 * TW) + 1;
            hx = r % (4 * TW) + 1;
            in_region = nb < NB;
        }
        const int b = b0 + nb, iy = iy0 + hy, ix = ix0 + hx;
        hpix[i] = 0;
        hoff[i] = SCRATCH;
        if (in_region && b < p.B && iy >= 0 && iy < p.Hin && ix >= 0 && ix < p.Win) {
            const int slot = (2 * hx + qd) ^ ((hx >> 3) & 1) ^ (((hy >> 2) & 3) << 1) ^ w4_nbcode(LTW, nb);
            hpix[i] = (b * p.Hin + iy) * p.Win + ix;
            hoff[i] = (nb * IH + hy) * RS + 4 * slot;
        }
    }
    f32x4 hreg[HR];
    const size_t in_px = (size_t)p.B * p.Hin * p.Win;
    const __amdgpu_buffer_rsrc_t rs_in0 = make_rsrc(p.in0, in_px * p.C0 * 4);
    const __amdgpu_buffer_rsrc_t rs_in1 = make_rsrc(p.C1 ? p.in1 : p.in0, in_px * (p.C1 ? p.C1 : p.C0) * 4);
    const unsigned hq = 4 * (tid & 1);
    unsigned hvo[HR];
    auto window_offsets = [&](unsigned Cs) {
#pragma unroll
        for (int i = 0; i < HR; ++i) hvo[i] = (__umul24((unsigned)hpix[i], Cs) + hq) * 4;
    };
    auto window_value = [&](int chunk, int i) {
        const bool s1 = chunk >= p.chunks0;
        return bufload4(s1 ? rs_in1 : rs_in0, hvo[i], (unsigned)(s1 ? chunk - p.chunks0 : chunk) * (W4CK * 4));
    };

    unsigned acol[5][2], aext[5];
    {
        const int tx = l15 & (TW - 1), ty = (l15 >> LTW) & (TH - 1), nb = l15 >> (2 * LTW);
#pragma unroll
        for (int cc = 0; cc < 5; ++cc) {
            const int c = cc == 0 ? (CT ? 5 : 0) : cc;
            const int hx = 4 * tx + c;
#pragma unroll
            for (int rhi = 0; rhi < 2; ++rhi) {
                const int slot = (2 * hx + (kq >> 1)) ^ ((hx >> 3) & 1) ^ (((ty + rhi) & 3) << 1) ^ w4_nbcode(LTW, nb);
                acol[cc][rhi] = (unsigned)(((nb * IH + 4 * ty) * RS + 4 * slot + 2 * (kq & 1)) * 4);
            }
            aext[cc] = acol[cc][RT] + (unsigned)((RT ? 5 : 0) * RS * 4);
        }
    }
    const char* sbytes = reinterpret_cast<const char*>(smem);
    auto rd2 = [&](unsigned byte_off) { return *reinterpret_cast<const f32x2*>(sbytes + byte_off); };
    const W4Coef cr = w4_coef(RT), cc_ = w4_coef(CT);

    const size_t u_chunk = (size_t)36 * p.Cout * W4CK;
    const __amdgpu_buffer_rsrc_t rs_w = make_rsrc(p.w, (size_t)p.n_chunks * u_chunk * 4);
    const unsigned uvo = (unsigned)((kq * 128 + l15 * 8) * 4);
    const unsigned u_slot = (unsigned)p.Cout * W4CK * 4;
    const unsigned u_wave = (unsigned)(9 * wave) * u_slot + (unsigned)n_tile * (64 * W4CK * 4);
    f32x4 U[9][2];
    auto load_u = [&](int chunk, int k) {
        const unsigned so = (unsigned)chunk * (unsigned)(u_chunk * 4) + u_wave + k * u_slot;
        U[k][0] = bufload4(rs_w, uvo, so);
        U[k][1] = bufload4(rs_w, uvo, so + 16);
    };

    f32x2 A[9];
    f32x4 acc[9][4];
    f32x2 T[3][5];

    auto row_stage_read = [&](auto bf_tag, auto cc_tag, f32x2 (&d)[5]) {
        constexpr int bf = decltype(bf_tag)::value, cc = decltype(cc_tag)::value;
        constexpr unsigned base = bf * BUF * 4;
        d[0] = rd2(aext[cc] + base);
        d[1] = rd2(acol[cc][0] + base + 1 * RS * 4);
        d[2] = rd2(acol[cc][0] + base + 2 * RS * 4);
        d[3] = rd2(acol[cc][0] + base + 3 * RS * 4);
        d[4] = rd2(acol[cc][1] + base + 4 * RS * 4);
    };
    auto row_stage_math = [&](int cc, const f32x2 (&d)[5]) {
        w4_half(cr, d[0], d[1], d[2], d[3], d[4], T[0][cc], T[1][cc], T[2][cc]);
    };
    auto col_stage = [&](int a) {
        w4_half(cc_, T[a][0], T[a][1], T[a][2], T[a][3], T[a][4], A[3 * a + 0], A[3 * a + 1], A[3 * a + 2]);
    };

    using I0 = std::integral_constant<int, 0>;
    using I1 = std::integral_constant<int, 1>;
    using I2 = std::integral_constant<int, 2>;
    using I3 = std::integral_constant<int, 3>;
    using I4 = std::integral_constant<int, 4>;

    f32x4 h2[HR];
    {
        const bool two = cb + 1 < ce;
        window_offsets(cb >= p.chunks0 ? p.C1 : p.C0);
#pragma unroll
        for (int i = 0; i < HR; ++i) hreg[i] = window_value(cb, i);
        const int c1 = two ? cb + 1 : cb;
        if (c1 == p.chunks0) window_offsets(p.C1);
#pragma unroll
        for (int i = 0; i < HR; ++i) h2[i] = window_value(c1, i);
#pragma unroll
        for (int k = 0; k < 9; ++k) load_u(cb, k);
    }
    {
        const f32x4 z4 = make_f32x4(0.f, 0.f, 0.f, 0.f);
        for (int i = tid; i < 2 * BUF / 4; i += 256) *reinterpret_cast<f32x4*>(smem + 4 * i) = z4;
        int* ptab = reinterpret_cast<int*>(smem + g.ptab_off);
        {
            const int i = tid;
            const int t = i >> 4, beta = (i >> 2) & 3, alpha = i & 3;
            const int tx = t & (TW - 1), ty = (t >> LTW) & (TH - 1), nb = t >> (2 * LTW);
            const int b = b0 + nb, y = 4 * (ty0 + ty) + alpha, x = 4 * (tx0 + tx) + beta;
            ptab[i] = (b < p.B && y < p.Ho && x < p.Wo) ? (b * p.Ho + y) * p.Wo + x : -1;
        }
    }

    __syncthreads();
    DM_STAMP_ADD(0)
#pragma unroll
    for (int i = 0; i < HR; ++i) *reinterpret_cast<f32x4*>(raw[0] + hoff[i]) = hreg[i];
#pragma unroll
    for (int i = 0; i < HR; ++i) *reinterpret_cast<f32x4*>(raw[1] + hoff[i]) = h2[i];
    __syncthreads();
    DM_STAMP_ADD(1)
    {
        f32x2 d[5];
        row_stage_read(I0{}, I0{}, d); row_stage_math(0, d);
        row_stage_read(I0{}, I1{}, d); row_stage_math(1, d);
        row_stage_read(I0{}, I2{}, d); row_stage_math(2, d);
        row_stage_read(I0{}, I3{}, d); row_stage_math(3, d);
        row_stage_read(I0{}, I4{}, d); row_stage_math(4, d);
#pragma unroll
        for (int a = 0; a < 3; ++a) col_stage(a);
    }
    __syncthreads();
    DM_STAMP_ADD(2)

    const f32x4 zero4 = make_f32x4(0.f, 0.f, 0.f, 0.f);
    auto chunk_body = [&](int c, auto first_tag, auto par_tag) {
        constexpr bool FIRST = decltype(first_tag)::value;
        constexpr int PAR = decltype(par_tag)::value;
        constexpr int BN = PAR ^ 1, BS = PAR;
        using BNT = std::integral_constant<int, BN>;
        const bool has1 = c + 1 < ce, has2 = c + 2 < ce;
        const int cw = has2 ? c + 2 : c;
        const int cun = has1 ? c + 1 : c;
        if (cw == p.chunks0 && p.C1 != p.C0) {
            window_offsets(p.C1);
            asm volatile("" ::: "memory");
        }
        f32x2 d[5];
#pragma unroll
        for (int k = 0; k < 9; ++k)
#pragma unroll
            for (int st = 0; st < 2; ++st)
#pragma unroll
                for (int gq = 0; gq < 4; ++gq) {
                    const int m = (k * 2 + st) * 4 + gq;
                    acc[k][gq] = __builtin_amdgcn_mfma_f32_16x16x4f32(A[k][st], U[k][gq >> 1][2 * (gq & 1) + st],
                                                                      (FIRST && st == 0) ? zero4 : acc[k][gq], 0, 0, 0);
                    if (m < HR) hreg[m] = window_value(cw, m);
                    if (m >= 60 && m < 60 + HR) *reinterpret_cast<f32x4*>(raw[BS] + hoff[m - 60]) = hreg[m - 60];
                    if (m == 8 * k + 7) load_u(cun, k);
                    if (m == 2) row_stage_read(BNT{}, I0{}, d);
                    if (m == 5) row_stage_math(0, d);
                    if (m == 8) row_stage_read(BNT{}, I1{}, d);
                    if (m == 11) row_stage_math(1, d);
                    if (m == 14) row_stage_read(BNT{}, I2{}, d);
                    if (m == 17) row_stage_math(2, d);
                    if (m == 20) row_stage_read(BNT{}, I3{}, d);
                    if (m == 23) row_stage_math(3, d);
                    if (m == 26) row_stage_read(BNT{}, I4{}, d);
                    if (m == 29) row_stage_math(4, d);
                    if (m == 32) col_stage(0);
                    if (m == 48) col_stage(1);
                    __builtin_amdgcn_sched_barrier(0);
                }
        col_stage(2);
        __syncthreads();
    };
    {
        using P0 = std::integral_constant<int, 0>;
        using P1 = std::integral_constant<int, 1>;
        chunk_body(cb, std::true_type{}, P0{});
        int c = cb + 1;
        for (; c + 1 < ce; c += 2) {
            chunk_body(c, std::false_type{}, P1{});
            chunk_body(c + 1, std::false_type{}, P0{});
        }
        if (c < ce) chunk_body(c, std::false_type{}, P1{});
    }

    DM_STAMP_ADD(3)
#pragma unroll
    for (int a = 0; a < 3; ++a)
#pragma unroll
        for (int gq = 0; gq < 4; ++gq) {
            const f32x4 vp = acc[3 * a + 1][gq], vm = acc[3 * a + 2][gq];
            acc[3 * a + 1][gq] = add4(vp, vm);
            acc[3 * a + 2][gq] = sub4(vp, vm);
        }
    const int c4 = l15 * 4;
    const int sub = lane >> 4;
    const int cg = n_tile * 64 + c4;
    const bool cvalid = cg < p.Cout;
    RowsEpilogue re;
    re.split = split;
    re.M = (size_t)p.B * p.Ho * p.Wo;
    re.b0 = b0;
    re.uni = NB == 1 || p.ss_stride == 0;
    re.HoWo = p.Ho * p.Wo;
    re.red = nullptr;
    re.rows_per_wg = 0;
    re.row_in_wg0 = 0;
    re.wn = 0;
    re.all_valid = true;
    const int* ptab = reinterpret_cast<const int*>(smem + g.ptab_off);
    const int my_tile = 4 * wave + sub;
    int pixv[2][8];
    RowsPrefetch<8, true> pf[2];
#pragma unroll
    for (int h = 0; h < 2; ++h) {
#pragma unroll
        for (int bb = 0; bb < 2; ++bb) {
            const int4 t4 = *reinterpret_cast<const int4*>(ptab + (my_tile * 4 + 2 * h + bb) * 4);
            pixv[h][4 * bb + 0] = t4.x;
            pixv[h][4 * bb + 1] = t4.y;
            pixv[h][4 * bb + 2] = t4.z;
            pixv[h][4 * bb + 3] = t4.w;
        }
        rows_prefetch<8, true>(p, re, pixv[h], cg, cvalid, pf[h]);
    }
    constexpr int RSZ = 12 * W4TILES * W4WTS;
    float* Rw = smem + (size_t)wave * 3 * W4TILES * W4WTS;
    auto beta_pair = [&](auto h_tag) {
        constexpr int h = decltype(h_tag)::value;
#pragma unroll
        for (int bb = 0; bb < 2; ++bb) {
            constexpr int beta0 = 2 * h;
            const int beta = beta0 + bb;
            const float c1 = CT ? (float)(1 << beta) : 1.0f;
            const float cP = CT ? (beta == 3 ? 1.0f : 0.0f) : (beta == 0 ? 1.0f : 0.0f);
            const f32x2 c12 = {c1, c1}, cP2 = {cP, cP};
#pragma unroll
            for (int a = 0; a < 3; ++a)
#pragma unroll
                for (int gq = 0; gq < 4; ++gq) {
                    const f32x4 x = acc[3 * a + 1 + bb][gq];
                    const f32x4 mp = acc[3 * a][gq];
                    const f32x4 r = join4(pk_fma(cP2, mp.xy, pk_mul(c12, x.xy)), pk_fma(cP2, mp.zw, pk_mul(c12, x.zw)));
                    float* dst = Rw + bb * RSZ + (a * W4TILES + 4 * kq) * W4WTS + 16 * gq + l15;
                    dst[0 * W4WTS] = r.x;
                    dst[1 * W4WTS] = r.y;
                    dst[2 * W4WTS] = r.z;
                    dst[3 * W4WTS] = r.w;
                }
        }
        __syncthreads();
        DM_STAMP_ADD(4)
        f32x4 v[8];
#pragma unroll
        for (int bb = 0; bb < 2; ++bb) {
            auto X = [&](int rt, int a) {
                const float* r0 = smem + bb * RSZ + ((size_t)((2 * rt + 0) * 3 + a) * W4TILES + my_tile) * W4WTS + c4;
                const float* r1 = smem + bb * RSZ + ((size_t)((2 * rt + 1) * 3 + a) * W4TILES + my_tile) * W4WTS + c4;
                return add4(*reinterpret_cast<const f32x4*>(r0), *reinterpret_cast<const f32x4*>(r1));
            };
            const f32x4 x0 = X(0, 0), x1 = X(0, 1), x2 = X(0, 2), x3 = X(1, 1), x4 = X(1, 2), x5 = X(1, 0);
            const f32x4 s12 = add4(x1, x2), d12 = sub4(x1, x2), s34 = add4(x3, x4), d34 = sub4(x3, x4);
            const f32x2 two = {2.f, 2.f}, four = {4.f, 4.f}, eight = {8.f, 8.f};
            v[4 * bb + 0] = add4(add4(x0, s12), s34);
            v[4 * bb + 1] = fma4(d34, two, d12);
            v[4 * bb + 2] = fma4(s34, four, s12);
            v[4 * bb + 3] = add4(fma4(d34, eight, d12), x5);
        }
        DM_STAMP_ADD(5)
        rows_epilogue<1, 8, true>(p, re, v, pixv[h], cg, cvalid, pf[h]);
        DM_STAMP_ADD(6)
    };
    beta_pair(I0{});
    __syncthreads();
    DM_STAMP_ADD(7)
    beta_pair(I1{});
    DM_STAMP_FLUSH
}

template <int LTW>
static int wino4_launch_t(const ConvParams& p, int blocks, hipStream_t s) {
    static LdsOptIn lds_flag;
    if (lds_opt_in(lds_flag, reinterpret_cast<const void*>(wino4_mfma_kernel<LTW>), 1)) return 1;
#ifdef DM_STAMPS
    {
        const size_t nblk = (size_t)blocks * p.geo.splits;
        unsigned long long* dbuf = nullptr;
        DM_CHECK_HIP(hipMalloc(reinterpret_cast<void**>(&dbuf), nblk * 8 * sizeof(unsigned long long)));
        DM_CHECK_HIP(hipMemsetAsync(dbuf, 0, nblk * 8 * sizeof(unsigned long long), s));
        ConvParams ps = p;
        ps.stamps = dbuf;
        hipLaunchKernelGGL(wino4_mfma_kernel<LTW>, dim3(blocks, p.geo.splits, 1), dim3(256), p.geo.lds_bytes, s, ps);
        DM_CHECK_HIP(hipStreamSynchronize(s));
        std::vector<unsigned long long> h(nblk * 8);
        DM_CHECK_HIP(hipMemcpy(h.data(), dbuf, h.size() * sizeof(unsigned long long), hipMemcpyDeviceToHost));
        (void)hipFree(dbuf);
        double avg[8] = {0};
        for (size_t b = 0; b < nblk; ++b)
            for (int k = 0; k < 8; ++k) avg[k] += (double)h[b * 8 + k] / nblk;
        fprintf(stderr, "STAMPS wino4<%d> %d+%d->%d @%dx%d e%d k%d chunks %d: wgs=%zu | setup %.0f loads->lds %.0f "
                        "transform0 %.0f loop %.0f (%.0f/chunk) stage1+bar %.0f final %.0f rows_epi %.0f midbar %.0f\n",
                LTW, p.C0, p.C1, p.Cout, p.Ho, p.Wo, p.epi, p.geo.splits, p.geo.chunks_per_split, nblk, avg[0], avg[1],
                avg[2], avg[3], avg[3] / p.geo.chunks_per_split, avg[4], avg[5], avg[6], avg[7]);
        return 0;
    }
#endif
    hipLaunchKernelGGL(wino4_mfma_kernel<LTW>, dim3(blocks, p.geo.splits, 1), dim3(256), p.geo.lds_bytes, s, p);
    DM_CHECK_HIP(hipGetLastError());
    return 0;
}

int wino4_launch(const ConvParams& pin, hipStream_t s) {
    ConvParams p = pin;
    p.stamps = nullptr;
    const ConvGeom& g = p.geo;
    DM_REQUIRE(p.KH == 3 && p.KW == 3 && p.stride == 1 && p.pad == 1 && !p.up && !p.fold, "winograd4: 3x3 s1 p1 only");
    DM_REQUIRE(!p.in_nchw && !p.out_nchw, "winograd4: NHWC only");
    DM_REQUIRE(p.C0 % W4CK == 0 && p.C1 % W4CK == 0 && p.Cout % 64 == 0, "winograd4: channel counts");
    DM_REQUIRE(p.Hin == p.Ho && p.Win == p.Wo, "winograd4: same-size convolution");
    const int ltw = w4_class(p.Ho, p.Wo);
    DM_REQUIRE(ltw >= 0 && ltw == g.lTW, "winograd4: image size has no geometry class");
    DM_REQUIRE(g.TW * g.TH * g.NB == W4TILES, "winograd4: 16 tiles per workgroup");
    DM_REQUIRE(4 * g.TW * g.tiles_x == p.Wo && 4 * g.TH * g.tiles_y == p.Ho, "winograd4: tiles must cover the image exactly");
    DM_REQUIRE((size_t)p.B * p.Ho * p.Wo < (1u << 24) && p.C0 < (1 << 24) && p.C1 < (1 << 24) &&
                   (size_t)p.B * p.Ho * p.Wo * std::max(p.C0, p.C1) < (1ull << 30),
               "winograd4: tensor too large for 24-bit pixel indices");
    DM_REQUIRE(!(p.epi & EPI_NORM) || (g.n_tiles_n == 1 && g.splits == 1), "winograd4: fused RMSNorm needs one N tile");
    DM_REQUIRE(g.splits == 1 || p.partial, "winograd4: split-K writes partial sums");
    DM_REQUIRE(g.lds_bytes <= 160 * 1024, "winograd4: tile does not fit LDS");
    DM_REQUIRE(p.chunks0 == p.C0 / W4CK && p.n_chunks == (p.C0 + p.C1) / W4CK, "winograd4: chunk counts");
    const int blocks = g.n_tiles_n * g.tiles_x * g.tiles_y * g.groups;
    p.geo.xcd_groups = (blocks % 8 == 0 && 8 % g.n_tiles_n == 0) ? 8 / g.n_tiles_n : 0;
    const bool timed = prof::enabled();
    if (timed) {
        const double pix = (double)p.B * p.Ho * p.Wo;
        const double cin = p.C0 + p.C1;
        const double flops = 2.0 * 9.0 * cin * p.Cout * pix;
        const double res_rows = (!p.partial && (p.epi & EPI_RESIDUAL)) ? 1.0 : 0.0;
        const double bytes = 4.0 * (cin * pix + (1.0 + res_rows) * p.Cout * pix + 9.0 * cin * p.Cout);
        char name[64];
        if (prof::detail())
            snprintf(name, sizeof(name), "wino4<%d> 3x3 s1 %d+%d->%d @%dx%d e%d k%d g%d", ltw, p.C0, p.C1, p.Cout, p.Ho, p.Wo,
                     p.epi, g.splits, blocks * g.splits);
        else
            snprintf(name, sizeof(name), "wino4_mfma_kernel<%d>", ltw);
        if (prof::begin(name, flops, bytes, s)) return 1;
    }
    int rc;
    switch (ltw) {
        case 0: rc = wino4_launch_t<0>(p, blocks, s); break;
        case 1: rc = wino4_launch_t<1>(p, blocks, s); break;
        default: rc = wino4_launch_t<2>(p, blocks, s); break;
    }
    if (rc) return 1;
    if (timed && prof::end(s)) return 1;
    return 0;
}

}
```

### include/dm_hip.h

```cpp
#ifndef DM_HIP_H
#define DM_HIP_H

#include <stdint.h>

#ifdef __cplusplus
extern "C" {
#endif

#define DM_MAX_STAGES 8

#define DM_TEXT_NONE 0
#define DM_TEXT_CONCAT 1
#define DM_TEXT_CROSS 2

typedef struct dm_unet_cfg {
    int32_t dim;
    int32_t init_dim;
    int32_t out_dim;
    int32_t channels;
    int32_t input_channels;
    int32_t n_stages;
    int32_t dim_mults[DM_MAX_STAGES];
    int32_t full_attn[DM_MAX_STAGES];
    int32_t attn_heads;
    int32_t attn_dim_head;
    int32_t text_mode;
    int32_t text_emb_dim;
    float sinusoidal_theta;
    int32_t learned_sinusoidal_dim;
    int32_t attn_heads_stage[DM_MAX_STAGES];
} dm_unet_cfg;

typedef struct dm_unet dm_unet;

const char* dm_last_error(void);
int dm_abi_version(void);


int dm_unet_create(const dm_unet_cfg* cfg, int device, dm_unet** out);
void dm_unet_destroy(dm_unet* u);

int dm_unet_set_param(dm_unet* u, const char* name, const float* data_host, const int64_t* shape, int ndim);
int dm_unet_missing_params(dm_unet* u);
int dm_unet_get_param_host(dm_unet* u, const char* name, float* out_host, int64_t n);
int dm_unet_finalize(dm_unet* u);

int dm_unet_update_param(dm_unet* u, const char* name, const float* data_host, const int64_t* shape, int ndim);
int dm_unet_refresh(dm_unet* u);
int dm_unet_graph_captures(dm_unet* u);
int64_t dm_unet_workspace_bytes(dm_unet* u);

int dm_unet_forward(dm_unet* u, const float* x, const int64_t* time, const float* ctx, int ctx_tokens,
                    float* out, int B, int H, int W, void* stream);

int dm_unet_forward_masked(dm_unet* u, const float* x, const int64_t* time, const float* ctx, int ctx_tokens,
                           const int32_t* text_mask, float* out, int B, int H, int W, void* stream);

#define DM_COEFS 8
#define DM_SAMPLER_DDPM 0
#define DM_SAMPLER_DDIM 1
#define DM_OBJ_PRED_NOISE 0
#define DM_OBJ_PRED_X0 1
#define DM_OBJ_PRED_V 2

int dm_sample(dm_unet* u, int kind, int n_steps, const int64_t* times_host, const float* coefs_host,
              const float* x_T, const float* noise, uint64_t seed, uint64_t sample_offset, const float* ctx,
              int ctx_tokens, float* out, float* all_steps, int B, int H, int W, int unnormalize, int use_graph,
              void* stream);

int dm_sample_cond(dm_unet* u, int kind, int n_steps, const int64_t* times_host, const float* coefs_host,
                   const float* x_T, const float* noise, uint64_t seed, uint64_t sample_offset, const float* ctx,
                   int ctx_tokens, const float* cond, int cond_channels, float* out, float* all_steps, int B, int H,
                   int W, int unnormalize, int use_graph, void* stream);

typedef struct dm_sample_args {
    int32_t kind;
    int32_t objective;
    int32_t self_condition;
    int32_t n_steps;
    const int64_t* times_host;
    const float* coefs_host;
    const float* x_T;
    const float* noise;
    uint64_t seed;
    uint64_t sample_offset;
    const float* ctx;
    int32_t ctx_tokens;
    int32_t cond_channels;
    const float* cond;
    float* out;
    float* all_steps;
    int32_t B, H, W;
    int32_t unnormalize;
    int32_t use_graph;
    int32_t reserved_;
    void* stream;
    int32_t cfg;
    float cfg_scale;
    float cfg_rescaled_phi;
    float cfg_keep_parallel_frac;
    int32_t cfg_remove_parallel;
    int32_t cfg_reserved_;
} dm_sample_args;
int dm_sample_ex(dm_unet* u, const dm_sample_args* args);

int dm_randn(float* out, int64_t n, uint64_t seed, uint64_t draw, uint64_t element_offset, void* stream);

typedef struct dm_decoder_cfg {
    int32_t ch;
    int32_t out_ch;
    int32_t n_levels;
    int32_t ch_mult[DM_MAX_STAGES];
    int32_t num_res_blocks;
    int32_t n_attn_res;
    int32_t attn_resolutions[DM_MAX_STAGES];
    int32_t resolution;
    int32_t z_channels;
    int32_t embed_dim;
} dm_decoder_cfg;

typedef struct dm_decoder dm_decoder;
int dm_decoder_create(const dm_decoder_cfg* cfg, int device, dm_decoder** out);
void dm_decoder_destroy(dm_decoder* d);
int dm_decoder_set_param(dm_decoder* d, const char* name, const float* data_host, const int64_t* shape, int ndim);
int dm_decoder_missing_params(dm_decoder* d);
int dm_decoder_finalize(dm_decoder* d);
int dm_decoder_forward(dm_decoder* d, const float* z, float* out, int B, int h, int w, void* stream);

typedef struct dm_encoder_cfg {
    int32_t ch;
    int32_t in_channels;
    int32_t n_levels;
    int32_t ch_mult[DM_MAX_STAGES];
    int32_t num_res_blocks;
    int32_t n_attn_res;
    int32_t attn_resolutions[DM_MAX_STAGES];
    int32_t resolution;
    int32_t z_channels;
    int32_t embed_dim;
    int32_t n_embed;
    int32_t double_z;
} dm_encoder_cfg;
typedef struct dm_encoder dm_encoder;
int dm_encoder_create(const dm_encoder_cfg* cfg, int device, dm_encoder** out);
void dm_encoder_destroy(dm_encoder* e);
int dm_encoder_set_param(dm_encoder* e, const char* name, const float* data_host, const int64_t* shape, int ndim);
int dm_encoder_missing_params(dm_encoder* e);
int dm_encoder_finalize(dm_encoder* e);
int dm_encoder_forward(dm_encoder* e, const float* x, float* zq, float* pre_quant, int32_t* indices, int B, int H, int W,
                       void* stream);


int dm_op_conv2d(const float* in0, int C0, const float* in1, int C1, const float* weight, const float* bias,
                 const float* residual, float* out, int B, int H, int W, int Cout, int ksize, int pad, int up2,
                 void* stream);
int dm_op_downsample(const float* in, int C, const float* weight, const float* bias, float* out, int B, int H,
                     int W, int Cout, void* stream);
int dm_op_rmsnorm(const float* x, const float* g, float* out, int B, int C, int H, int W, void* stream);
int dm_op_block(const float* x, int Cin, const float* weight, const float* bias, const float* g,
                const float* scale, const float* shift, float* out, int B, int H, int W, int Cout, void* stream);
int dm_op_linear_attention(const float* x, const float* norm_g, const float* mem_kv, const float* w_qkv,
                           const float* w_out, const float* b_out, const float* out_g, float* out, int B, int C,
                           int H, int W, int heads, int dim_head, void* stream);
int dm_op_attention(const float* x, const float* norm_g, const float* mem_kv, const float* w_qkv,
                    const float* w_out, const float* b_out, float* out, int B, int C, int H, int W, int heads,
                    int dim_head, void* stream);
int dm_op_sampler_update(int kind, int objective, const float* x, const float* eps, const float* noise,
                         const float* c_host, float* out, float* x_start, int64_t n, void* stream);
int dm_op_cfg_combine(const float* cond, const float* null_out, float* out, int B, int64_t per_sample, float cond_scale,
                      float rescaled_phi, int remove_parallel_component, float keep_parallel_frac, void* stream);
int dm_op_group_norm(const float* x_nhwc, const float* weight, const float* bias, float* y_nhwc, int B, int HW, int C,
                     int groups, float eps, int swish, void* stream);
int dm_op_vae_attention(const float* q, const float* k, const float* v, float* out, int B, int n, int C, int kernel,
                        void* stream);
int dm_op_vq_nearest(const float* z_rows, const float* codebook, float* zq_nchw, int32_t* indices, int64_t pixels, int E,
                     int n_embed, int hw, void* stream);

typedef struct dm_conv dm_conv;
int dm_conv_create(const float* weight_host, const float* bias_host, int Cout, int Cin, int KH, int KW, int stride,
                   int pad_h, int pad_w, int relu, int device, dm_conv** out);
void dm_conv_destroy(dm_conv* c);
int dm_conv_forward(dm_conv* c, const float* in, int in_nchw, int B, int H, int W, float* out_nhwc, void* stream);
int dm_op_pool2d(const float* in, float* out, int B, int H, int W, int C, int k, int stride, int pad, int mode,
                 void* stream);
int dm_op_resize_bilinear(const float* in_nchw, float* out_nhwc, int B, int C, int H, int W, int Ho, int Wo,
                          const float* scale_dev, const float* shift_dev, void* stream);
int dm_op_copy_channels_nhwc(const float* src, int Cs, float* dst, int Cd, int c_off, int64_t rows, void* stream);
int dm_op_global_avgpool(const float* in_nhwc, float* out, int B, int HW, int C, void* stream);
int dm_op_linear(const float* x, const float* weight, const float* bias, float* y, int R, int I, int O, void* stream);


int dm_unet_train_enable(dm_unet* u);
int64_t dm_unet_grad_floats(dm_unet* u);
int dm_unet_grads_flat(dm_unet* u, float** ptr_out, int64_t* n_out);
int dm_unet_train_buckets(dm_unet* u, int enable);
int dm_unet_train_bucket(dm_unet* u, int i, int64_t* off_out, int64_t* n_out, int wait, void* wait_stream);
int dm_unet_get_grad(dm_unet* u, const char* name, float* out_dev, void* stream);
int dm_unet_loss_backward(dm_unet* u, const float* x_start, const int64_t* t_host, const float* coef_host,
                          const float* noise, const float* noise_q, const float* cond, int cond_channels, const float* ctx,
                          int ctx_tokens,
                          int self_cond, int objective, float loss_scale, int accumulate, float* loss_out_host,
                          float* model_out, int B, int H, int W, void* stream);
typedef struct dm_train_args {
    const float* x_start;
    const int64_t* t_host;
    const float* coef_host;
    int coef_stride;
    const float* noise;
    const float* noise_q;
    const float* cond;
    int cond_channels;
    const float* ctx;
    int ctx_tokens;
    int self_cond;
    int objective;
    float loss_scale;
    int accumulate;
    float* loss_out_host;
    float* model_out;
    int B, H, W;
    void* stream;
    int loss_terms;
    float kl_scale;
} dm_train_args;
int dm_unet_loss_backward_ex(dm_unet* u, const dm_train_args* a);
int dm_unet_loss_backward_masked(dm_unet* u, const dm_train_args* a, const int32_t* text_mask);
int dm_unet_optimizer_step(dm_unet* u, double lr, double beta1, double beta2, double eps, float max_grad_norm,
                           float* grad_norm_out_host, void* stream);
int dm_unet_train_scalar(dm_unet* u, int which, float* out_dev, void* stream);
int dm_unet_ema_update(dm_unet* u, double decay, int copy, void* stream);
int dm_unet_get_param(dm_unet* u, const char* name, int which, float* out_dev, void* stream);
int dm_unet_set_train_tensor(dm_unet* u, const char* name, int which, const float* src_dev, void* stream);
long long dm_unet_adam_step(dm_unet* u, long long set_to);
int dm_unet_train_sync(dm_unet* u);
int dm_unet_check_device_pack(dm_unet* u);
int dm_unet_train_dropout(dm_unet* u, float p, uint64_t seed);
int dm_op_dropout_mask(float* out, int64_t n, float p, uint64_t seed, uint64_t call, int block_index, void* stream);
int dm_op_q_sample(const float* x_start, const float* noise, const float* coef_host, float* out, int B, int per_sample,
                   void* stream);
int dm_op_lincomb(const float* x, const float* y, const float* coef_host, float* out, int B, int64_t per_sample, int mode,
                  int clamp, void* stream);
int dm_op_mask_mix(const float* a, const float* b, const float* mask, float* out, int64_t n, void* stream);
int dm_op_offset_noise(float* noise, const float* offset, float strength, int BC, int HW, void* stream);
int dm_op_cdist(const float* x, const float* y, float* out, int n, int m, int64_t D, void* stream);
int dm_op_gather_rows(const float* src, const int64_t* idx_host, float* dst, int n, int64_t D, void* stream);
int dm_op_mse_loss(const float* out, const float* x_start, const float* noise, const float* xq, const float* coef_host,
                   int objective, int terms, float loss_scale, float kl_weight, float* dout, float* loss_out_host,
                   float* part_out, float* klpart_out, int B, int per_sample, void* stream);
int dm_op_adam_step(float* p, const float* g, float* m, float* v, int64_t n, double lr, double beta1, double beta2, double eps,
                    int step, float max_grad_norm, float* norm_coef_out_host, void* stream);
int dm_op_ema_lerp(float* ema, const float* p, int64_t n, double decay, void* stream);

int dm_op_conv2d_bwd(const float* in0, int C0, const float* in1, int C1, const float* weight, const float* dy, float* d_in0,
                     float* d_in1, float* d_weight, float* d_bias, int B, int H, int W, int Cout, int ksize, int pad, int up2,
                     void* stream);
int dm_op_downsample_bwd(const float* in, int C, const float* weight, const float* dy, float* d_in, float* d_weight,
                         float* d_bias, int B, int H, int W, int Cout, void* stream);
int dm_op_block_bwd(const float* x, int Cin, const float* weight, const float* bias, const float* g, const float* scale,
                    const float* shift, const float* dy, float* dx, float* d_weight, float* d_bias, float* d_g,
                    float* d_scale, float* d_shift, int B, int H, int W, int Cout, void* stream);
int dm_op_linear_bwd(const float* x, const float* weight, const float* dy, float* dx, float* d_weight, float* d_bias, int R,
                     int I, int O, int accumulate, void* stream);
int dm_op_rmsnorm_bwd(const float* x, const float* g, const float* dy, float* dx, float* dg, int B, int C, int H, int W,
                      void* stream);
int dm_op_linear_attention_bwd(const float* x, const float* norm_g, const float* mem_kv, const float* w_qkv,
                               const float* w_out, const float* b_out, const float* out_g, const float* dy, float* dx,
                               float* d_norm_g, float* d_mem_kv, float* d_w_qkv, float* d_w_out, float* d_b_out,
                               float* d_out_g, int B, int C, int H, int W, int heads, int dim_head, void* stream);
int dm_op_attention_bwd(const float* x, const float* norm_g, const float* mem_kv, const float* w_qkv, const float* w_out,
                        const float* b_out, const float* dy, float* dx, float* d_norm_g, float* d_mem_kv, float* d_w_qkv,
                        float* d_w_out, float* d_b_out, int B, int C, int H, int W, int heads, int dim_head, void* stream);
int dm_op_cross_attention(const float* x, const float* ctx, const float* w_q, const float* w_k, const float* w_v,
                          const float* w_out, const float* b_out, const float* out_g, const int32_t* text_mask, float* out,
                          int B, int C, int H, int W, int m, int E, int dim_head, void* stream);
int dm_op_cross_attention_bwd(const float* x, const float* ctx, const float* w_q, const float* w_k, const float* w_v,
                              const float* w_out, const float* b_out, const float* out_g, const int32_t* text_mask,
                              const float* dy, float* y_out, float* dx, float* d_w_q, float* d_w_k, float* d_w_v,
                              float* d_w_out, float* d_b_out, float* d_out_g, int B, int C, int H, int W, int m, int E,
                              int dim_head, void* stream);

typedef struct dm_profile_row {
    char kernel[64];
    int64_t launches;
    double total_ms;
    double total_flops;
    double total_bytes;
} dm_profile_row;
int dm_profile_enable(int on);
int dm_profile_read(dm_profile_row* rows, int max_rows, int* n_rows);

int dm_unet_forward_ft(dm_unet* u, const float* x, const float* time, const float* ctx, int ctx_tokens, float* out, int B,
                       int H, int W, void* stream);

#define DM_EDM_COEFS 16
#define DM_EDM_HEUN 0
#define DM_EDM_DPMPP 1
typedef struct dm_edm_args {
    int32_t kind;
    int32_t n_steps;
    const float* table_host;
    const float* x_init;
    const float* noise;
    uint64_t seed;
    uint64_t sample_offset;
    float* out;
    float sigma_init;
    int32_t clamp;
    int32_t B, H, W;
    int32_t use_graph;
    void* stream;
} dm_edm_args;
int dm_sample_edm(dm_unet* u, const dm_edm_args* args);

int dm_op_edm_churn_in(const float* x, const float* eps, const float* c_host, int rows, uint64_t seed, uint64_t draw,
                       uint64_t element_offset, float* xhat, float* xin, int B, int64_t per, void* stream);
int dm_op_edm_euler(const float* xhat, const float* F, const float* c_host, int rows, int clamp, float* D_out, float* d_out,
                    float* xnext, float* xin_next, int B, int64_t per, void* stream);
int dm_op_edm_heun(const float* xhat, const float* d, const float* xnext, const float* F2, const float* c_host, int rows,
                   int clamp, float* out, int B, int64_t per, void* stream);
int dm_op_edm_dpmpp(const float* x, const float* F, float* d_old, const float* c_host, int rows, float* out, int B,
                    int64_t per, void* stream);
int dm_op_edm_finalize(const float* x, float* out, int64_t n, void* stream);

int dm_unet_train_enable_ft(dm_unet* u, int time_weights_frozen);

typedef struct dm_edm_train_args {
    const float* images;
    const float* noise;
    const float* coef_host;
    int32_t coef_stride;
    float loss_scale;
    int32_t accumulate;
    int32_t B, H, W;
    float* loss_out_host;
    float* denoised_out;
    void* stream;
} dm_edm_train_args;
int dm_unet_loss_backward_edm(dm_unet* u, const dm_edm_train_args* args);

int dm_op_edm_noise_in(const float* images, const float* eps, const float* c_host, int rows, float* x0, float* noised,
                       float* xin, int B, int64_t per, void* stream);
int dm_op_edm_loss(const float* noised, const float* F, const float* x0, const float* c_host, float loss_scale, float* dF,
                   float* D_out, float* loss_out_host, int B, int64_t per, void* stream);
int dm_op_sinusoid_ft_bwd(const float* de0, const float* e0, float* dw, int B, int half, int learned, int accumulate,
                          void* stream);

#define DM_CT_COEFS 16
#define DM_CT_PRED_NOISE 0
#define DM_CT_PRED_V 1
typedef struct dm_ct_args {
    int32_t objective;
    int32_t clip;
    int32_t n_steps;
    const float* table_host;
    const float* x_init;
    const float* noise;
    uint64_t seed;
    uint64_t sample_offset;
    float* out;
    int32_t B, H, W;
    int32_t use_graph;
    void* stream;
} dm_ct_args;
int dm_sample_ct(dm_unet* u, const dm_ct_args* args);

typedef struct dm_ct_train_args {
    const float* images;
    const float* noise;
    const float* coef_host;
    int32_t coef_stride;
    int32_t objective;
    float loss_scale;
    int32_t accumulate;
    int32_t B, H, W;
    int32_t normalize;
    float* loss_out_host;
    void* stream;
} dm_ct_train_args;
int dm_unet_loss_backward_ct(dm_unet* u, const dm_ct_train_args* args);

int dm_op_ct_step(const float* x, const float* F, const float* eps, const float* c_host, int rows, int objective, int clip,
                  uint64_t seed, uint64_t draw, uint64_t element_offset, float* out, float* x_start_out, int B, int64_t per,
                  void* stream);
int dm_op_ct_noise_in(const float* images, const float* eps, const float* c_host, int rows, int objective, int normalize,
                      float* x, float* target, int B, int64_t per, void* stream);
int dm_op_ct_loss(const float* F, const float* target, const float* c_host, float loss_scale, float* dF,
                  float* loss_out_host, int B, int64_t per, void* stream);

#ifdef __cplusplus
}
#endif
#endif
```

Baseline: 57.18 images/s.

## Pre-transform Winograd F(4x4) input tiles once when many output-channel tiles reuse them

Adds a separate kernel that computes the Winograd input transform (V) once per input tile and chunk and stores it in a workspace buffer. The main MFMA kernel gains a PRE variant that streams V directly from memory instead of staging halos in LDS and transforming them. This path is enabled when there are at least four output-channel tiles, so the transform is no longer redone for each of them. The cost is an extra launch, a large V buffer and extra global traffic, and the path is disabled during training.

```diff
diff --git a/diffusion-models_amd/_lib.py b/diffusion-models_amd/_lib.py
--- a/diffusion-models_amd/_lib.py
+++ b/diffusion-models_amd/_lib.py
@@ -23,7 +23,7 @@
     "dm_decoder_finalize", "dm_decoder_forward",
     "dm_encoder_create", "dm_encoder_destroy", "dm_encoder_set_param", "dm_encoder_missing_params",
     "dm_encoder_finalize", "dm_encoder_forward",
-    "dm_op_conv2d", "dm_op_downsample", "dm_op_rmsnorm", "dm_op_block", "dm_op_linear_attention",
+    "dm_op_conv2d", "dm_op_wino4_xform", "dm_op_downsample", "dm_op_rmsnorm", "dm_op_block", "dm_op_linear_attention",
     "dm_op_attention", "dm_op_sampler_update", "dm_op_cfg_combine",
     "dm_op_group_norm", "dm_op_vae_attention", "dm_op_vq_nearest",
     "dm_conv_create", "dm_conv_destroy", "dm_conv_forward", "dm_op_pool2d", "dm_op_resize_bilinear",
@@ -172,6 +172,7 @@
     lib.dm_encoder_finalize.argtypes = [vp]
     lib.dm_encoder_forward.argtypes = [vp, fp, fp, fp, vp, i32, i32, i32, vp]
     lib.dm_op_conv2d.argtypes = [fp, i32, fp, i32, fp, fp, fp, fp, i32, i32, i32, i32, i32, i32, i32, vp]
+    lib.dm_op_wino4_xform.argtypes = [fp, i32, fp, i32, fp, C.c_int64, i32, i32, i32, vp]
     lib.dm_op_downsample.argtypes = [fp, i32, fp, fp, fp, i32, i32, i32, i32, vp]
     lib.dm_op_rmsnorm.argtypes = [fp, fp, fp, i32, i32, i32, i32, vp]
     lib.dm_op_block.argtypes = [fp, i32, fp, fp, fp, fp, fp, fp, i32, i32, i32, i32, vp]
diff --git a/diffusion-models_amd/csrc/conv_device.h b/diffusion-models_amd/csrc/conv_device.h
--- a/diffusion-models_amd/csrc/conv_device.h
+++ b/diffusion-models_amd/csrc/conv_device.h
@@ -65,6 +65,10 @@
 }
 __device__ __forceinline__ f32x4 bufload4(__amdgpu_buffer_rsrc_t r, unsigned voff_bytes, unsigned soff_bytes) {
     return __builtin_bit_cast(f32x4, __builtin_amdgcn_raw_buffer_load_b128(r, (int)voff_bytes, (int)soff_bytes, 0));
+}
+
+__device__ __forceinline__ f32x2 bufload2(__amdgpu_buffer_rsrc_t r, unsigned voff_bytes, unsigned soff_bytes) {
+    return __builtin_bit_cast(f32x2, __builtin_amdgcn_raw_buffer_load_b64(r, (int)voff_bytes, (int)soff_bytes, 0));
 }
 
 __device__ __forceinline__ float fast_rcp(float x) { return __builtin_amdgcn_rcpf(x); }
diff --git a/diffusion-models_amd/csrc/dm_api.hip b/diffusion-models_amd/csrc/dm_api.hip
--- a/diffusion-models_amd/csrc/dm_api.hip
+++ b/diffusion-models_amd/csrc/dm_api.hip
@@ -855,6 +855,7 @@
         p.chunks0 = L.C0 / 8;
         p.n_chunks = (L.C0 + L.C1) / 8;
         p.geo = wino4_plan(c.B, p.Ho, p.Wo, L.Cout, L.C0, L.C1, true);
+        if (c.u && c.u->train) p.geo.pre = 0;
         P.kind = 2;
     } else if (wino) {
         p.w = L.ww;
@@ -877,6 +878,11 @@
         case 1: return wino_launch(q, s);
         default: return conv_launch(q, s);
     }
+}
+
+static float* alloc_vpre(Ctx& c, PlannedConv& P) {
+    if (P.kind != 2 || !P.p.geo.pre) return nullptr;
+    return P.p.vpre = c.A->alloc(wino4_v_floats(P.p.geo, P.p.n_chunks));
 }
 
 static int run_conv(Ctx& c, const ConvLayer& L, const float* in0, const float* in1, int Hin, int Win, float* out,
@@ -896,19 +902,28 @@
     const int full_epi = epi | (L.bias ? EPI_BIAS : 0);
     if (P.in_kernel) {
         DM_REQUIRE(!res_parts, "residual partial sums need the landing pass");
-        if (c.dry()) return 0;
+        float* v = alloc_vpre(c, P);
+        if (c.dry()) {
+            c.A->release(v);
+            return 0;
+        }
         p.out = out; p.partial = 0; p.epi = full_epi;
-        return launch_planned(P, p, c.s, c.u);
+        const int rc = launch_planned(P, p, c.s, c.u);
+        c.A->release(v);
+        return rc;
     }
     DM_REQUIRE(!out_nchw, "split / unfused epilogue writes NHWC");
     const size_t M = (size_t)c.B * P.out_h * P.out_w;
     float* part = c.A->alloc((size_t)p.geo.splits * M * L.Cout);
+    float* v = alloc_vpre(c, P);
     if (c.dry()) {
+        c.A->release(v);
         c.A->release(part);
         return 0;
     }
     p.out = part; p.partial = 1; p.epi = 0;
     if (launch_planned(P, p, c.s, c.u)) return 1;
+    c.A->release(v);
     int rc;
     if (res_parts)
         rc = launch_norm_act(part, p.geo.splits, (int64_t)(M * L.Cout), L.bias, g, scale, c.ss_stride, P.out_h * P.out_w,
@@ -931,9 +946,15 @@
     const size_t M = (size_t)c.B * P.out_h * P.out_w;
     *part = c.A->alloc((size_t)p.geo.splits * M * L.Cout);
     *nsplit = p.geo.splits;
-    if (c.dry()) return 0;
+    float* v = alloc_vpre(c, P);
+    if (c.dry()) {
+        c.A->release(v);
+        return 0;
+    }
     p.out = *part; p.partial = 1; p.epi = 0;
-    return launch_planned(P, p, c.s, c.u);
+    const int rc = launch_planned(P, p, c.s, c.u);
+    c.A->release(v);
+    return rc;
 }
 
 static int run_block(Ctx& c, const ConvLayer& L, const float* in0, const float* in1, int H, int W, const float* g,
diff --git a/diffusion-models_amd/csrc/dm_common.h b/diffusion-models_amd/csrc/dm_common.h
--- a/diffusion-models_amd/csrc/dm_common.h
+++ b/diffusion-models_amd/csrc/dm_common.h
@@ -79,11 +79,13 @@
     int lds_bytes;
     int xcd_groups;
     int NQ;
+    int pre;
 };
 
 struct ConvParams {
     const float* in0;
     const float* in1;
+    float* vpre;
     int C0, C1;
     int chunks0;
     int n_chunks;
@@ -130,6 +132,8 @@
 void wino4_pack_weights(const float* oihw, float* packed, int Cout, int C0, int C1);
 ConvGeom wino4_plan(int B, int Ho, int Wo, int Cout, int C0, int C1, bool allow_split);
 bool wino4_shape_ok(int B, int Ho, int Wo, int Cout, int C0, int C1);
+size_t wino4_v_floats(const ConvGeom& g, int n_chunks);
+int wino4_xform_launch(const ConvParams& p, float* v, hipStream_t s);
 int wino4_launch(const ConvParams& p, hipStream_t s);
 
 bool init7_eligible(int Cout, int C0, int C1, int KH, int KW, int stride, int pad, bool up);
diff --git a/diffusion-models_amd/csrc/dm_ops.inc b/diffusion-models_amd/csrc/dm_ops.inc
--- a/diffusion-models_amd/csrc/dm_ops.inc
+++ b/diffusion-models_amd/csrc/dm_ops.inc
@@ -78,6 +78,34 @@
     });
 }
 
+int dm_op_wino4_xform(const float* in0, int C0, const float* in1, int C1, float* v, int64_t v_floats, int B, int H, int W,
+                      void* stream) {
+    DM_REQUIRE(in0 && v, "null argument");
+    DM_REQUIRE(C0 > 0 && C0 % 8 == 0 && C1 % 8 == 0, "channel counts must be multiples of 8");
+    DM_REQUIRE((H == 4 && W == 4) || (H == 8 && W == 8) || (H > 0 && W > 0 && H % 16 == 0 && W % 16 == 0),
+               "image size has no F(4x4) geometry class");
+    hipStream_t s = static_cast<hipStream_t>(stream);
+    if (!in1) C1 = 0;
+    ConvParams p{};
+    p.C0 = C0; p.C1 = C1;
+    p.chunks0 = C0 / 8; p.n_chunks = (C0 + C1) / 8;
+    p.B = B; p.Hin = H; p.Win = W; p.Ho = H; p.Wo = W;
+    p.geo = wino4_plan(B, H, W, 64, C0, C1, false);
+    DM_REQUIRE((size_t)v_floats == wino4_v_floats(p.geo, p.n_chunks), "v_floats does not match the V layout of this shape");
+    return run_op(s, [&](Arena& A) -> int {
+        int rc = 0;
+        float* a0 = to_nhwc(A, in0, B, C0, H * W, s, &rc);
+        float* a1 = in1 ? to_nhwc(A, in1, B, C1, H * W, s, &rc) : nullptr;
+        float* vv = A.alloc((size_t)v_floats);
+        if (rc) return 1;
+        if (A.dry) return 0;
+        p.in0 = a0; p.in1 = a1;
+        if (wino4_xform_launch(p, vv, s)) return 1;
+        DM_CHECK_HIP(hipMemcpyAsync(v, vv, (size_t)v_floats * sizeof(float), hipMemcpyDeviceToDevice, s));
+        return 0;
+    });
+}
+
 int dm_op_downsample(const float* in, int C, const float* weight, const float* bias, float* out, int B, int H,
                      int W, int Cout, void* stream) {
     DM_REQUIRE(in && weight && out, "null argument");
diff --git a/diffusion-models_amd/csrc/wino4_mfma.hip b/diffusion-models_amd/csrc/wino4_mfma.hip
--- a/diffusion-models_amd/csrc/wino4_mfma.hip
+++ b/diffusion-models_amd/csrc/wino4_mfma.hip
@@ -34,6 +34,12 @@
 }
 
 size_t wino4_packed_floats(int Cout, int C0, int C1) { return (size_t)(C0 + C1) * 36 * Cout; }
+
+static constexpr int W4VW = 9 * 64 * 2;
+static constexpr int W4_PRE_MIN_TILES = 4;
+size_t wino4_v_floats(const ConvGeom& g, int n_chunks) {
+    return (size_t)n_chunks * g.tiles_x * g.tiles_y * g.groups * 4 * W4VW;
+}
 
 static inline int w4_index(int h, int t) {
     static const int lo[3] = {0, 1, 2}, hi[3] = {5, 3, 4};
@@ -104,6 +110,7 @@
     g.splits = (n_chunks + g.chunks_per_split - 1) / g.chunks_per_split;
     g.fused_norm = g.n_tiles_n == 1 && g.splits == 1;
     g.w_floats = 0;
+    g.pre = ltw >= 0 && g.n_tiles_n >= W4_PRE_MIN_TILES && wino4_v_floats(g, n_chunks) < (size_t(1) << 29);
     g.ptab_off = std::max(3 * g.halo_floats + 16, 2 * 12 * W4TILES * W4WTS);
     g.lds_bytes = (g.ptab_off + 16 * W4TILES) * 4;
     return g;
@@ -164,7 +171,7 @@
     oP = pk_fma_s(c.p3, z3, t);
 }
 
-template <int LTW>
+template <int LTW, bool PRE>
 __global__ __launch_bounds__(256, 1) void wino4_mfma_kernel(const ConvParams p) {
     using G = W4Geo<LTW>;
     constexpr int TW = G::TW, TH = G::TH, NB = G::NB, IH = G::IH, IW = G::IW, RS = G::RS, BUF = G::BUF, HR = G::HR;
@@ -179,6 +186,7 @@
 
     int n_tile, bid;
     block_to_tile(g, blockIdx.x, gridDim.x, n_tile, bid);
+    const int pblock = bid;
     const int tile_x = bid % g.tiles_x;
     bid /= g.tiles_x;
     const int tile_y = bid % g.tiles_y;
@@ -268,6 +276,19 @@
         U[k][1] = bufload4(rs_w, uvo, so + 16);
     };
 
+    const unsigned n_pb = gridDim.x / (unsigned)g.n_tiles_n;
+    const __amdgpu_buffer_rsrc_t rs_v = make_rsrc(PRE ? p.vpre : p.in0, PRE ? (size_t)p.n_chunks * n_pb * (4 * W4VW * 4) : 0);
+    f32x4 AP[2][4];
+    f32x2 AL[2];
+    auto load_v = [&](int chunk, auto set_tag, int j) {
+        constexpr int set = decltype(set_tag)::value;
+        const unsigned so = (((unsigned)chunk * n_pb + (unsigned)pblock) * 4 + (unsigned)wave) * (W4VW * 4);
+        if (j < 4)
+            AP[set][j] = bufload4(rs_v, (unsigned)lane * 16 + j * 1024, so);
+        else
+            AL[set] = bufload2(rs_v, (unsigned)lane * 8 + 4096, so);
+    };
+
     f32x2 A[9];
     f32x4 acc[9][4];
     f32x2 T[3][5];
@@ -295,7 +316,12 @@
     using I4 = std::integral_constant<int, 4>;
 
     f32x4 h2[HR];
-    {
+    if constexpr (PRE) {
+#pragma unroll
+        for (int j = 0; j < 5; ++j) load_v(cb, std::integral_constant<int, 0>{}, j);
+#pragma unroll
+        for (int k = 0; k < 9; ++k) load_u(cb, k);
+    } else {
         const bool two = cb + 1 < ce;
         window_offsets(cb >= p.chunks0 ? p.C1 : p.C0);
 #pragma unroll
@@ -308,8 +334,10 @@
         for (int k = 0; k < 9; ++k) load_u(cb, k);
     }
     {
-        const f32x4 z4 = make_f32x4(0.f, 0.f, 0.f, 0.f);
-        for (int i = tid; i < 2 * BUF / 4; i += 256) *reinterpret_cast<f32x4*>(smem + 4 * i) = z4;
+        if constexpr (!PRE) {
+            const f32x4 z4 = make_f32x4(0.f, 0.f, 0.f, 0.f);
+            for (int i = tid; i < 2 * BUF / 4; i += 256) *reinterpret_cast<f32x4*>(smem + 4 * i) = z4;
+        }
         int* ptab = reinterpret_cast<int*>(smem + g.ptab_off);
         {
             const int i = tid;
@@ -322,13 +350,13 @@
 
     __syncthreads();
     DM_STAMP_ADD(0)
-#pragma unroll
-    for (int i = 0; i < HR; ++i) *reinterpret_cast<f32x4*>(raw[0] + hoff[i]) = hreg[i];
-#pragma unroll
-    for (int i = 0; i < HR; ++i) *reinterpret_cast<f32x4*>(raw[1] + hoff[i]) = h2[i];
-    __syncthreads();
-    DM_STAMP_ADD(1)
-    {
+    if constexpr (!PRE) {
+#pragma unroll
+        for (int i = 0; i < HR; ++i) *reinterpret_cast<f32x4*>(raw[0] + hoff[i]) = hreg[i];
+#pragma unroll
+        for (int i = 0; i < HR; ++i) *reinterpret_cast<f32x4*>(raw[1] + hoff[i]) = h2[i];
+        __syncthreads();
+        DM_STAMP_ADD(1)
         f32x2 d[5];
         row_stage_read(I0{}, I0{}, d); row_stage_math(0, d);
         row_stage_read(I0{}, I1{}, d); row_stage_math(1, d);
@@ -337,9 +365,9 @@
         row_stage_read(I0{}, I4{}, d); row_stage_math(4, d);
 #pragma unroll
         for (int a = 0; a < 3; ++a) col_stage(a);
-    }
-    __syncthreads();
-    DM_STAMP_ADD(2)
+        __syncthreads();
+        DM_STAMP_ADD(2)
+    }
 
     const f32x4 zero4 = make_f32x4(0.f, 0.f, 0.f, 0.f);
     auto chunk_body = [&](int c, auto first_tag, auto par_tag) {
@@ -350,9 +378,11 @@
         const bool has1 = c + 1 < ce, has2 = c + 2 < ce;
         const int cw = has2 ? c + 2 : c;
         const int cun = has1 ? c + 1 : c;
-        if (cw == p.chunks0 && p.C1 != p.C0) {
-            window_offsets(p.C1);
-            asm volatile("" ::: "memory");
+        if constexpr (!PRE) {
+            if (cw == p.chunks0 && p.C1 != p.C0) {
+                window_offsets(p.C1);
+                asm volatile("" ::: "memory");
+            }
         }
         f32x2 d[5];
 #pragma unroll
@@ -362,8 +392,19 @@
 #pragma unroll
                 for (int gq = 0; gq < 4; ++gq) {
                     const int m = (k * 2 + st) * 4 + gq;
-                    acc[k][gq] = __builtin_amdgcn_mfma_f32_16x16x4f32(A[k][st], U[k][gq >> 1][2 * (gq & 1) + st],
+                    float a_op;
+                    if constexpr (PRE)
+                        a_op = k < 8 ? AP[PAR][k >> 1][2 * (k & 1) + st] : AL[PAR][st];
+                    else
+                        a_op = A[k][st];
+                    acc[k][gq] = __builtin_amdgcn_mfma_f32_16x16x4f32(a_op, U[k][gq >> 1][2 * (gq & 1) + st],
                                                                       (FIRST && st == 0) ? zero4 : acc[k][gq], 0, 0, 0);
+                    if constexpr (PRE) {
+                        if (m < 5) load_v(cun, BNT{}, m);
+                        if (m == 8 * k + 7) load_u(cun, k);
+                        __builtin_amdgcn_sched_barrier(0);
+                        continue;
+                    }
                     if (m < HR) hreg[m] = window_value(cw, m);
                     if (m >= 60 && m < 60 + HR) *reinterpret_cast<f32x4*>(raw[BS] + hoff[m - 60]) = hreg[m - 60];
                     if (m == 8 * k + 7) load_u(cun, k);
@@ -381,8 +422,10 @@
                     if (m == 48) col_stage(1);
                     __builtin_amdgcn_sched_barrier(0);
                 }
-        col_stage(2);
-        __syncthreads();
+        if constexpr (!PRE) {
+            col_stage(2);
+            __syncthreads();
+        }
     };
     {
         using P0 = std::integral_constant<int, 0>;
@@ -490,10 +533,155 @@
     DM_STAMP_FLUSH
 }
 
+static constexpr int W4XC = 4;
+
+struct W4XformParams {
+    const float* in0;
+    const float* in1;
+    int C0, C1, chunks0, n_chunks;
+    int B, H, W, tiles_x, tiles_y, n_pb;
+    float* v;
+};
+
 template <int LTW>
+__global__ __launch_bounds__(256) void wino4_xform_kernel(const W4XformParams p) {
+    using G = W4Geo<LTW>;
+    constexpr int TW = G::TW, TH = G::TH, NB = G::NB, IH = G::IH, IW = G::IW, RS = G::RS, BUF = G::BUF, HR = G::HR;
+    __shared__ __attribute__((aligned(16))) float smem[BUF + 16];
+    const int tid = threadIdx.x;
+    const int lane = tid & 63;
+    const int wave = __builtin_amdgcn_readfirstlane(tid >> 6);
+    const int RT = wave >> 1, CT = wave & 1;
+    const int l15 = lane & 15, kq = lane >> 4;
+    int bid = blockIdx.x;
+    const int tile_x = bid % p.tiles_x;
+    bid /= p.tiles_x;
+    const int tile_y = bid % p.tiles_y;
+    const int group = bid / p.tiles_y;
+    const int ix0 = 4 * tile_x * TW - 1, iy0 = 4 * tile_y * TH - 1, b0 = group * NB;
+    const int cb = blockIdx.y * W4XC;
+    const int ce = min(cb + W4XC, p.n_chunks);
+
+    int hpix[HR], hoff[HR];
+#pragma unroll
+    for (int i = 0; i < HR; ++i) {
+        const int it = tid + 256 * i;
+        const int hp = it >> 1, qd = it & 1;
+        int nb, hy, hx;
+        bool in_region;
+        if constexpr (LTW == 2) {
+            hy = hp / IW;
+            hx = hp - hy * IW;
+            nb = 0;
+            in_region = hp < IH * IW;
+        } else {
+            constexpr int PIX = 16 * TW * TH;
+            nb = hp / PIX;
+            const int r = hp - nb * PIX;
+            hy = r / (4 * TW) + 1;
+            hx = r % (4 * TW) + 1;
+            in_region = nb < NB;
+        }
+        const int b = b0 + nb, iy = iy0 + hy, ix = ix0 + hx;
+        hpix[i] = 0;
+        hoff[i] = BUF;
+        if (in_region && b < p.B && iy >= 0 && iy < p.H && ix >= 0 && ix < p.W) {
+            const int slot = (2 * hx + qd) ^ ((hx >> 3) & 1) ^ (((hy >> 2) & 3) << 1) ^ w4_nbcode(LTW, nb);
+            hpix[i] = (b * p.H + iy) * p.W + ix;
+            hoff[i] = (nb * IH + hy) * RS + 4 * slot;
+        }
+    }
+    const size_t in_px = (size_t)p.B * p.H * p.W;
+    const __amdgpu_buffer_rsrc_t rs_in0 = make_rsrc(p.in0, in_px * p.C0 * 4);
+    const __amdgpu_buffer_rsrc_t rs_in1 = make_rsrc(p.C1 ? p.in1 : p.in0, in_px * (p.C1 ? p.C1 : p.C0) * 4);
+    const unsigned hq = 4 * (tid & 1);
+    f32x4 hreg[W4XC][HR];
+#pragma unroll
+    for (int n = 0; n < W4XC; ++n) {
+        const int c = min(cb + n, ce - 1);
+        const bool s1 = c >= p.chunks0;
+        const unsigned Cs = s1 ? p.C1 : p.C0;
+#pragma unroll
+        for (int i = 0; i < HR; ++i)
+            hreg[n][i] = bufload4(s1 ? rs_in1 : rs_in0, (__umul24((unsigned)hpix[i], Cs) + hq) * 4,
+                                  (unsigned)(s1 ? c - p.chunks0 : c) * (W4CK * 4));
+    }
+    {
+        const f32x4 z4 = make_f32x4(0.f, 0.f, 0.f, 0.f);
+        for (int i = tid; i < BUF / 4; i += 256) *reinterpret_cast<f32x4*>(smem + 4 * i) = z4;
+    }
+
+    unsigned acol[5][2], aext[5];
+    {
+        const int tx = l15 & (TW - 1), ty = (l15 >> LTW) & (TH - 1), nb = l15 >> (2 * LTW);
+#pragma unroll
+        for (int cc = 0; cc < 5; ++cc) {
+            const int c = cc == 0 ? (CT ? 5 : 0) : cc;
+            const int hx = 4 * tx + c;
+#pragma unroll
+            for (int rhi = 0; rhi < 2; ++rhi) {
+                const int slot = (2 * hx + (kq >> 1)) ^ ((hx >> 3) & 1) ^ (((ty + rhi) & 3) << 1) ^ w4_nbcode(LTW, nb);
+                acol[cc][rhi] = (unsigned)(((nb * IH + 4 * ty) * RS + 4 * slot + 2 * (kq & 1)) * 4);
+            }
+            aext[cc] = acol[cc][RT] + (unsigned)((RT ? 5 : 0) * RS * 4);
+        }
+    }
+    const char* sbytes = reinterpret_cast<const char*>(smem);
+    auto rd2 = [&](unsigned byte_off) { return *reinterpret_cast<const f32x2*>(sbytes + byte_off); };
+    const W4Coef cr = w4_coef(RT), cc_ = w4_coef(CT);
+    float* vw = p.v + ((size_t)blockIdx.x * 4 + wave) * W4VW;
+    const size_t v_chunk = (size_t)p.n_pb * 4 * W4VW;
+
+    __syncthreads();
+#pragma unroll
+    for (int n = 0; n < W4XC; ++n) {
+        if (cb + n >= ce) break;
+#pragma unroll
+        for (int i = 0; i < HR; ++i) *reinterpret_cast<f32x4*>(smem + hoff[i]) = hreg[n][i];
+        __syncthreads();
+        f32x2 T[3][5], A[9];
+#pragma unroll
+        for (int cc = 0; cc < 5; ++cc) {
+            const f32x2 d0 = rd2(aext[cc]);
+            const f32x2 d1 = rd2(acol[cc][0] + 1 * RS * 4);
+            const f32x2 d2 = rd2(acol[cc][0] + 2 * RS * 4);
+            const f32x2 d3 = rd2(acol[cc][0] + 3 * RS * 4);
+            const f32x2 d4 = rd2(acol[cc][1] + 4 * RS * 4);
+            w4_half(cr, d0, d1, d2, d3, d4, T[0][cc], T[1][cc], T[2][cc]);
+        }
+#pragma unroll
+        for (int a = 0; a < 3; ++a)
+            w4_half(cc_, T[a][0], T[a][1], T[a][2], T[a][3], T[a][4], A[3 * a + 0], A[3 * a + 1], A[3 * a + 2]);
+        __syncthreads();
+        float* vc = vw + (size_t)(cb + n) * v_chunk;
+#pragma unroll
+        for (int j = 0; j < 4; ++j) *reinterpret_cast<f32x4*>(vc + j * 256 + lane * 4) = join4(A[2 * j], A[2 * j + 1]);
+        *reinterpret_cast<f32x2*>(vc + 1024 + lane * 2) = A[8];
+    }
+}
+
+template <int LTW>
+static int wino4_xform_launch_t(const W4XformParams& x, hipStream_t s) {
+    hipLaunchKernelGGL(wino4_xform_kernel<LTW>, dim3(x.n_pb, (x.n_chunks + W4XC - 1) / W4XC, 1), dim3(256), 0, s, x);
+    DM_CHECK_HIP(hipGetLastError());
+    return 0;
+}
+
+int wino4_xform_launch(const ConvParams& p, float* v, hipStream_t s) {
+    const ConvGeom& g = p.geo;
+    W4XformParams x{p.in0, p.in1, p.C0, p.C1, p.chunks0, p.n_chunks, p.B, p.Hin, p.Win, g.tiles_x, g.tiles_y,
+                    g.tiles_x * g.tiles_y * g.groups, v};
+    switch (g.lTW) {
+        case 0: return wino4_xform_launch_t<0>(x, s);
+        case 1: return wino4_xform_launch_t<1>(x, s);
+        default: return wino4_xform_launch_t<2>(x, s);
+    }
+}
+
+template <int LTW, bool PRE>
 static int wino4_launch_t(const ConvParams& p, int blocks, hipStream_t s) {
     static LdsOptIn lds_flag;
-    if (lds_opt_in(lds_flag, reinterpret_cast<const void*>(wino4_mfma_kernel<LTW>), 1)) return 1;
+    if (lds_opt_in(lds_flag, reinterpret_cast<const void*>(wino4_mfma_kernel<LTW, PRE>), 1)) return 1;
 #ifdef DM_STAMPS
     {
         const size_t nblk = (size_t)blocks * p.geo.splits;
@@ -502,7 +690,7 @@
         DM_CHECK_HIP(hipMemsetAsync(dbuf, 0, nblk * 8 * sizeof(unsigned long long), s));
         ConvParams ps = p;
         ps.stamps = dbuf;
-        hipLaunchKernelGGL(wino4_mfma_kernel<LTW>, dim3(blocks, p.geo.splits, 1), dim3(256), p.geo.lds_bytes, s, ps);
+        hipLaunchKernelGGL((wino4_mfma_kernel<LTW, PRE>), dim3(blocks, p.geo.splits, 1), dim3(256), p.geo.lds_bytes, s, ps);
         DM_CHECK_HIP(hipStreamSynchronize(s));
         std::vector<unsigned long long> h(nblk * 8);
         DM_CHECK_HIP(hipMemcpy(h.data(), dbuf, h.size() * sizeof(unsigned long long), hipMemcpyDeviceToHost));
@@ -510,14 +698,14 @@
         double avg[8] = {0};
         for (size_t b = 0; b < nblk; ++b)
             for (int k = 0; k < 8; ++k) avg[k] += (double)h[b * 8 + k] / nblk;
-        fprintf(stderr, "STAMPS wino4<%d> %d+%d->%d @%dx%d e%d k%d chunks %d: wgs=%zu | setup %.0f loads->lds %.0f "
+        fprintf(stderr, "STAMPS wino4<%d>%s %d+%d->%d @%dx%d e%d k%d chunks %d: wgs=%zu | setup %.0f loads->lds %.0f "
                         "transform0 %.0f loop %.0f (%.0f/chunk) stage1+bar %.0f final %.0f rows_epi %.0f midbar %.0f\n",
-                LTW, p.C0, p.C1, p.Cout, p.Ho, p.Wo, p.epi, p.geo.splits, p.geo.chunks_per_split, nblk, avg[0], avg[1],
+                LTW, PRE ? " pre" : "", p.C0, p.C1, p.Cout, p.Ho, p.Wo, p.epi, p.geo.splits, p.geo.chunks_per_split, nblk, avg[0], avg[1],
                 avg[2], avg[3], avg[3] / p.geo.chunks_per_split, avg[4], avg[5], avg[6], avg[7]);
         return 0;
     }
 #endif
-    hipLaunchKernelGGL(wino4_mfma_kernel<LTW>, dim3(blocks, p.geo.splits, 1), dim3(256), p.geo.lds_bytes, s, p);
+    hipLaunchKernelGGL((wino4_mfma_kernel<LTW, PRE>), dim3(blocks, p.geo.splits, 1), dim3(256), p.geo.lds_bytes, s, p);
     DM_CHECK_HIP(hipGetLastError());
     return 0;
 }
@@ -541,6 +729,7 @@
     DM_REQUIRE(g.splits == 1 || p.partial, "winograd4: split-K writes partial sums");
     DM_REQUIRE(g.lds_bytes <= 160 * 1024, "winograd4: tile does not fit LDS");
     DM_REQUIRE(p.chunks0 == p.C0 / W4CK && p.n_chunks == (p.C0 + p.C1) / W4CK, "winograd4: chunk counts");
+    DM_REQUIRE(!g.pre || p.vpre, "winograd4: the pre-transformed path needs its V buffer");
     const int blocks = g.n_tiles_n * g.tiles_x * g.tiles_y * g.groups;
     p.geo.xcd_groups = (blocks % 8 == 0 && 8 % g.n_tiles_n == 0) ? 8 / g.n_tiles_n : 0;
     const bool timed = prof::enabled();
@@ -552,17 +741,21 @@
         const double bytes = 4.0 * (cin * pix + (1.0 + res_rows) * p.Cout * pix + 9.0 * cin * p.Cout);
         char name[64];
         if (prof::detail())
-            snprintf(name, sizeof(name), "wino4<%d> 3x3 s1 %d+%d->%d @%dx%d e%d k%d g%d", ltw, p.C0, p.C1, p.Cout, p.Ho, p.Wo,
-                     p.epi, g.splits, blocks * g.splits);
+            snprintf(name, sizeof(name), "wino4<%d> 3x3 s1 %d+%d->%d @%dx%d e%d k%d g%d%s", ltw, p.C0, p.C1, p.Cout, p.Ho,
+                     p.Wo, p.epi, g.splits, blocks * g.splits, g.pre ? " pre" : "");
         else
-            snprintf(name, sizeof(name), "wino4_mfma_kernel<%d>", ltw);
+            snprintf(name, sizeof(name), "wino4_mfma_kernel<%d%s>", ltw, g.pre ? ",pre" : "");
         if (prof::begin(name, flops, bytes, s)) return 1;
     }
+    if (g.pre && wino4_xform_launch(p, p.vpre, s)) return 1;
     int rc;
-    switch (ltw) {
-        case 0: rc = wino4_launch_t<0>(p, blocks, s); break;
-        case 1: rc = wino4_launch_t<1>(p, blocks, s); break;
-        default: rc = wino4_launch_t<2>(p, blocks, s); break;
+    switch (ltw + (g.pre ? 3 : 0)) {
+        case 0: rc = wino4_launch_t<0, false>(p, blocks, s); break;
+        case 1: rc = wino4_launch_t<1, false>(p, blocks, s); break;
+        case 2: rc = wino4_launch_t<2, false>(p, blocks, s); break;
+        case 3: rc = wino4_launch_t<0, true>(p, blocks, s); break;
+        case 4: rc = wino4_launch_t<1, true>(p, blocks, s); break;
+        default: rc = wino4_launch_t<2, true>(p, blocks, s); break;
     }
     if (rc) return 1;
     if (timed && prof::end(s)) return 1;
diff --git a/include/dm_hip.h b/include/dm_hip.h
--- a/include/dm_hip.h
+++ b/include/dm_hip.h
@@ -154,6 +154,8 @@
 int dm_op_conv2d(const float* in0, int C0, const float* in1, int C1, const float* weight, const float* bias,
                  const float* residual, float* out, int B, int H, int W, int Cout, int ksize, int pad, int up2,
                  void* stream);
+int dm_op_wino4_xform(const float* in0, int C0, const float* in1, int C1, float* v, int64_t v_floats, int B, int H, int W,
+                      void* stream);
 int dm_op_downsample(const float* in, int C, const float* weight, const float* bias, float* out, int B, int H,
                      int W, int Cout, void* stream);
 int dm_op_rmsnorm(const float* x, const float* g, float* out, int B, int C, int H, int W, void* stream);
```

Result: no change. 56.84 images/s (-0.6%).
